# AbeelLab/phasm

Measured on AMD Instinct MI355X. Metric: overlaps_per_sec, higher is better.
Workload: dtype u64

## Files before the change

### include/phasm_overlap.h

```cpp
#ifndef PHASM_OVERLAP_H
#define PHASM_OVERLAP_H

#include <stddef.h>
#include <stdint.h>

#ifdef __cplusplus
extern "C" {
#endif

#define PO_ABI_VERSION 4

typedef enum {
    PO_OK = 0,
    PO_ERR_INVALID = 1,
    PO_ERR_NOMEM = 2,
    PO_ERR_HIP = 3,
    PO_ERR_CAPACITY = 4
} po_status;

typedef struct po_handle po_handle;
typedef struct po_result po_result;

typedef struct {
    uint32_t a_idx, b_idx;
// ... 417 lines not shown
    uint64_t n_invalid;
    uint64_t n_excluded;
    uint64_t n_root_starts;
    uint64_t n_late_starts;
    uint64_t n_blocked;
    uint64_t n_covered_edges, n_uncovered_edges;
    uint64_t n_paths;
    uint64_t n_short_paths;
    uint64_t n_isolated;
    uint64_t n_short_isolated;
    uint64_t n_contigs;
    uint64_t max_path_nodes;
    uint64_t n_chains;
    uint32_t n_path_rounds, n_cover_rounds;
    uint32_t n_batches;
    uint32_t reserved;
    float ms_ranks, ms_bubblechains, ms_paths, ms_cover, ms_label, ms_total;
} po_contig_stats;

po_status po_layout_contigs(po_handle* h, po_result* graph, const po_contig_params* params, const uint8_t* exclude_in,
                            uint32_t* edge_contig_out, uint32_t* edge_pos_out, po_contig* contigs_out, uint64_t* n_contigs_out);
po_status po_get_contig_stats(const po_handle* h, po_contig_stats* out);


typedef struct {
    uint32_t ploidy;
    uint32_t n_paths;
    uint32_t n_cands;
    uint32_t n_reads;
    uint32_t n_b;
    uint32_t start_of_block;
    uint32_t min_spanning_reads;
    uint32_t prune;
    uint32_t max_candidates;
    uint32_t n_levels;
    double threshold;
    uint32_t reserved;
    uint32_t reserved2;
} po_phase_params;

typedef struct {
    const int32_t* overlap_max;
    const uint32_t* aln_off;
    const uint32_t* aln_b;
    const int32_t* aln_a0;
    const int32_t* aln_a1;
    const uint32_t* path_off;
    const uint32_t* path_ids;
    const uint32_t* set_off;
    const uint32_t* set_ids;
    const double* levels;
} po_phase_input;

typedef struct {
    uint64_t n_extensions;
    uint64_t n_kept;
    uint64_t n_survivors;
    uint64_t level_counts[16];
    double max_rl;
    int32_t level_used;
    uint32_t n_levels;
    float ms_intervals, ms_table, ms_extend, ms_filter, ms_prune, ms_total;
} po_phase_stats;

po_status po_phase_branch(po_handle* h, const po_phase_params* params, const po_phase_input* input, uint32_t* cand_out,
                          uint32_t* ext_out, double* rl_out, uint64_t cap, double* table_out, uint64_t* n_out);
po_status po_get_phase_stats(const po_handle* h, po_phase_stats* out);


typedef struct {
    uint32_t b;
    int32_t a0, a1;
    uint32_t seq;
} po_alignment;

typedef struct {
    uint64_t n_rows, n_keys, max_degree, n_invalid;
    float ms_insert, ms_fill, ms_place, ms_total;
} po_phase_index_stats;

po_status po_phase_index(po_handle* h, po_result* rows, po_result** index_out);
po_status po_phase_index_copy(po_result* index, uint64_t* off_out, po_alignment* entries_out, uint64_t cap, uint64_t* n_out);
po_status po_get_phase_index_stats(const po_handle* h, po_phase_index_stats* out);

typedef struct {
    uint32_t mode;
    uint32_t min_spanning_reads;
    uint32_t reserved, reserved2;
} po_relevant_params;

typedef struct {
    const uint32_t* cur_graph;     uint64_t n_cur_graph;
    const uint32_t* prev_graph;    uint64_t n_prev_graph;
    const uint32_t* prev_aligning; uint64_t n_prev_aligning;
    const uint32_t* pred_read; const int32_t* pred_edge_len; uint64_t n_pred;
} po_relevant_input;

typedef struct {
    uint64_t n_cur_aligning, n_spanning, n_relevant, n_alignments, n_b;
    uint32_t fell_back, reserved;
} po_relevant_dims;

typedef struct {
    uint64_t n_cur_aligning, n_spanning, n_relevant, n_alignments, n_b;
    uint32_t fell_back, reserved;
    float ms_mark, ms_lists, ms_alignments, ms_total;
} po_relevant_stats;

po_status po_phase_relevant(po_handle* h, po_result* index, const po_relevant_params* params, const po_relevant_input* input,
                            po_result** out);
po_status po_relevant_sizes(const po_result* out, po_relevant_dims* sizes);
po_status po_relevant_copy(po_result* out, uint32_t* cur_aligning, uint32_t* rel_reads, int32_t* overlap_max, uint32_t* aln_off,
                           uint32_t* aln_b, int32_t* aln_a0, int32_t* aln_a1, uint32_t* b_reads);
po_status po_get_relevant_stats(const po_handle* h, po_relevant_stats* out);

typedef struct {
    uint64_t n_seqs, n_pieces;
    const uint64_t* seq_off;
    const uint32_t* piece_read;
    const uint32_t* piece_take;
} po_spell_input;

typedef struct {
    uint64_t n_seqs, n_pieces, n_bytes;
    uint64_t n_patched;
    float device_ms;
    uint32_t reserved;
} po_spell_stats;

po_status po_spell(po_handle* h, const po_spell_input* in, po_result** out);
po_status po_spell_sizes(const po_result* out, uint64_t* n_seqs, uint64_t* n_bytes);
po_status po_spell_copy(po_result* out, uint64_t* seq_byte_off, uint8_t* bytes, uint64_t cap);
po_status po_get_spell_stats(const po_handle* h, po_spell_stats* out);

po_status po_graph_from_edges(po_handle* h, const po_edge* edges, uint64_t n_edges, const uint32_t* node_order,
                              uint64_t n_order, po_result** out);

po_status po_result_node_order(po_result* r, uint32_t* nodes_out, uint64_t cap, uint64_t* n_out);

typedef struct {
    uint64_t n_rows;
    float ms_first_contained;
    float ms_rank;
    float ms_total;
} po_node_order_stats;
po_status po_get_node_order_stats(const po_handle* h, po_node_order_stats* out);

uint64_t po_debug_host_ranges(uint64_t* out, uint64_t cap_entries);
uint64_t po_debug_store_words(const po_handle* h, int store, const uint64_t** words);
int po_debug_expand_records(const po_cand* records, uint64_t n, const uint32_t* lengths, uint32_t n_reads, uint32_t paired,
                            po_row* rows_out, uint64_t n_rows_expected);
int po_debug_expand_packed(const uint64_t* records, uint64_t n, uint32_t sh_b, uint32_t sh_p, const uint32_t* lengths, uint32_t n_reads,
                           uint32_t paired, po_row* rows_out, uint64_t n_rows_expected);
int po_debug_fault_backtrace(int fd);
int po_debug_pointer_info(const void* p, int32_t* hip_type, int32_t* hsa_type, uint64_t* base, uint64_t* bytes);

po_status po_get_stats(const po_handle* h, po_stats* out);
const char* po_last_error(const po_handle* h);
int po_abi_version(void);

#ifdef __cplusplus
}
#endif
#endif
```

### phasm_amd/_lib.py

```python
from __future__ import annotations

import ctypes
import os

import numpy as np

HERE = os.path.dirname(os.path.abspath(__file__))
LIB_PATH = os.environ.get("PHASM_LIB") or os.path.join(HERE, "libphasm_overlap.so")

PO_OK, PO_ERR_INVALID, PO_ERR_NOMEM, PO_ERR_HIP, PO_ERR_CAPACITY = range(5)

ROW_DTYPE = np.dtype([("a_idx", "<u4"), ("b_idx", "<u4"), ("astart", "<i4"),
                      ("aend", "<i4"), ("bstart", "<i4"), ("bend", "<i4")])


CAND_DTYPE = np.dtype([("a_idx", "<u4"), ("p", "<u4"), ("b_idx", "<u4"), ("type", "<u4")])


EDGE_DTYPE = np.dtype([("u", "<u4"), ("v", "<u4"), ("weight", "<i4"), ("overlap_len", "<i4")])
COVERAGE_DTYPE = np.dtype([("read_length_sum", "<u8"), ("path_length", "<i8")])
COMPONENT_DTYPE = np.dtype([("first_node", "<u4"), ("n_nodes", "<u4"), ("n_edges", "<u8")])
SCC_DTYPE = np.dtype([("first_node", "<u4"), ("n_nodes", "<u4"), ("n_edges", "<u8"), ("n_r_in", "<u4"), ("n_re_out", "<u4")])
PART_R_IN, PART_RE_OUT, PART_START, PART_SINK = 1, 2, 4, 8
SUPERBUBBLE_DTYPE = np.dtype([("entrance", "<u4"), ("exit", "<u4"), ("n_inside", "<u4"), ("nested", "<u4")])
# ... 237 lines not shown
        return {name: getattr(self, name) for name, _ in self._fields_ if name != "reserved"}


class PoSpellInput(ctypes.Structure):
    _fields_ = [("n_seqs", ctypes.c_uint64), ("n_pieces", ctypes.c_uint64), ("seq_off", ctypes.c_void_p), ("piece_read", ctypes.c_void_p),
                ("piece_take", ctypes.c_void_p)]


class PoSpellStats(ctypes.Structure):
    _fields_ = [(name, ctypes.c_uint64) for name in ("n_seqs", "n_pieces", "n_bytes", "n_patched")] + \
               [("device_ms", ctypes.c_float), ("reserved", ctypes.c_uint32)]

    def as_dict(self) -> dict:
        return {name: getattr(self, name) for name, _ in self._fields_ if name != "reserved"}


class PoNodeOrderStats(ctypes.Structure):
    _fields_ = [("n_rows", ctypes.c_uint64), ("ms_first_contained", ctypes.c_float), ("ms_rank", ctypes.c_float),
                ("ms_total", ctypes.c_float)]

    def as_dict(self) -> dict:
        return {name: getattr(self, name) for name, _ in self._fields_}


class PoStats(ctypes.Structure):
    _fields_ = [
        ("bits_per_base", ctypes.c_uint32), ("kmer", ctypes.c_uint32),
        ("paired", ctypes.c_uint32), ("wide_index", ctypes.c_uint32),
        ("n_reads", ctypes.c_uint64), ("n_eligible", ctypes.c_uint64),
        ("total_bases", ctypes.c_uint64), ("shard_bases", ctypes.c_uint64),
        ("n_tiles", ctypes.c_uint64), ("n_candidates", ctypes.c_uint64),
        ("n_verified", ctypes.c_uint64), ("n_rows", ctypes.c_uint64),
        ("sum_overlap_bases", ctypes.c_uint64), ("verify_bytes_algo", ctypes.c_uint64),
        ("ms_index", ctypes.c_float), ("ms_scan_count", ctypes.c_float),
        ("ms_scan_fill", ctypes.c_float), ("ms_verify", ctypes.c_float),
        ("ms_select", ctypes.c_float), ("ms_emit", ctypes.c_float),
        ("ms_total", ctypes.c_float), ("ms_upload", ctypes.c_float),
        ("ms_scan_probe", ctypes.c_float), ("ms_verify_kernel", ctypes.c_float),
        ("verify_bytes_exec", ctypes.c_uint64), ("dp_steps", ctypes.c_uint64), ("dp_stopped", ctypes.c_uint64),
        ("max_diff", ctypes.c_uint32), ("band", ctypes.c_uint32), ("index_reused", ctypes.c_uint32),
        ("dp_lanes", ctypes.c_uint32), ("upload_bytes", ctypes.c_uint64),
        ("streamed", ctypes.c_uint32), ("n_deferred", ctypes.c_uint32),
        ("fused_tail", ctypes.c_uint32), ("tail_fallback", ctypes.c_uint32),
        ("n_predicted", ctypes.c_uint32), ("home_record_bytes", ctypes.c_uint32),
    ]

    def as_dict(self) -> dict:
        return {name: getattr(self, name) for name, _ in self._fields_}


_P = ctypes.c_void_p
SYMBOLS = [
    ("po_abi_version", ctypes.c_int, []),
    ("po_create", ctypes.c_int, [ctypes.POINTER(_P)]),
    ("po_destroy", None, [_P]),
    ("po_set_device", ctypes.c_int, [_P, ctypes.c_int]),
    ("po_add_sequence", ctypes.c_int, [_P, ctypes.c_char_p, ctypes.c_size_t, ctypes.c_char_p, ctypes.c_size_t]),
    ("po_add_fasta", ctypes.c_int, [_P, ctypes.c_char_p, ctypes.c_int, ctypes.POINTER(ctypes.c_uint64)]),
    ("po_num_sequences", ctypes.c_uint32, [_P]),
    ("po_get_id", ctypes.c_int, [_P, ctypes.c_uint32, ctypes.POINTER(ctypes.c_void_p), ctypes.POINTER(ctypes.c_size_t)]),
    ("po_get_length", ctypes.c_uint32, [_P, ctypes.c_uint32]),
    ("po_upload", ctypes.c_int, [_P]),
    ("po_invalidate", ctypes.c_int, [_P]),
    ("po_upload_piece", ctypes.c_int, [_P, ctypes.c_uint32, ctypes.c_uint32, ctypes.c_void_p, ctypes.c_uint64,
                                       ctypes.POINTER(ctypes.c_uint64), ctypes.POINTER(ctypes.c_int)]),
    ("po_upload_assemble", ctypes.c_int, [_P, ctypes.c_void_p, ctypes.c_uint64, ctypes.c_uint32]),
    ("po_upload_piece_part", ctypes.c_int, [_P, ctypes.c_uint32, ctypes.c_uint32, ctypes.c_uint32, ctypes.c_uint32, ctypes.c_void_p,
                                            ctypes.c_uint64, ctypes.POINTER(ctypes.c_uint64), ctypes.POINTER(ctypes.c_int)]),
    ("po_upload_assemble_parts", ctypes.c_int, [_P, ctypes.c_void_p, ctypes.c_uint64, ctypes.c_uint32, ctypes.c_uint32]),
    ("po_overlaps", ctypes.c_int, [_P, ctypes.c_uint32, ctypes.POINTER(_P)]),
    ("po_overlaps_to_host", ctypes.c_int, [_P, ctypes.c_uint32, ctypes.POINTER(_P)]),
    ("po_overlaps_ex", ctypes.c_int, [_P, ctypes.c_uint32, ctypes.c_uint32, ctypes.c_uint32, ctypes.POINTER(_P)]),
    ("po_overlaps_shard", ctypes.c_int, [_P, ctypes.c_uint32, ctypes.c_uint32, ctypes.c_uint32, ctypes.POINTER(_P)]),
    ("po_candidates_shard", ctypes.c_int, [_P, ctypes.c_uint32, ctypes.c_uint32, ctypes.c_uint32, ctypes.POINTER(_P)]),
    ("po_expand", ctypes.c_int, [_P, ctypes.c_void_p, ctypes.c_uint64, ctypes.POINTER(_P)]),
    ("po_candidates_shard_into", ctypes.c_int, [_P, ctypes.c_uint32, ctypes.c_uint32, ctypes.c_uint32, ctypes.c_void_p,
                                               ctypes.c_uint64, ctypes.POINTER(ctypes.c_int), ctypes.POINTER(_P)]),
    ("po_index_slice_build", ctypes.c_int, [_P, ctypes.c_uint32, ctypes.c_uint32, ctypes.c_uint32, ctypes.POINTER(ctypes.c_uint32),
                                            ctypes.POINTER(ctypes.c_uint32), ctypes.POINTER(ctypes.c_uint64)]),
    ("po_index_chunk_bytes", ctypes.c_uint64, [ctypes.c_uint32, ctypes.c_uint64, ctypes.POINTER(ctypes.c_uint64)]),
    ("po_index_slice_export", ctypes.c_int, [_P, ctypes.c_void_p, ctypes.c_uint64]),
    ("po_candidates_shard_indexed", ctypes.c_int, [_P, ctypes.c_uint32, ctypes.c_uint32, ctypes.c_uint32, ctypes.c_void_p, ctypes.c_uint32,
                                                   ctypes.c_uint32, ctypes.c_uint64, ctypes.c_void_p, ctypes.c_uint64,
                                                   ctypes.POINTER(ctypes.c_int), ctypes.POINTER(_P)]),
    ("po_overlaps_shard_indexed", ctypes.c_int, [_P, ctypes.c_uint32, ctypes.c_uint32, ctypes.c_uint32, ctypes.c_void_p, ctypes.c_uint32,
                                                 ctypes.c_uint32, ctypes.c_uint64, ctypes.POINTER(_P)]),
    ("po_shard_range", ctypes.c_int, [_P, ctypes.c_uint32, ctypes.c_uint32, ctypes.POINTER(ctypes.c_uint32), ctypes.POINTER(ctypes.c_uint32)]),
    ("po_result_count", ctypes.c_uint64, [_P]),
    ("po_result_rows", ctypes.c_void_p, [_P]),
    ("po_result_rows_range", ctypes.c_void_p, [_P, ctypes.c_uint64, ctypes.c_uint64]),
    ("po_result_device_rows", ctypes.c_void_p, [_P]),
    ("po_result_copy_to_device", ctypes.c_int, [_P, ctypes.c_void_p]),
    ("po_result_copy_prefix_to_device", ctypes.c_int, [_P, ctypes.c_void_p, ctypes.c_uint64]),
    ("po_result_free", None, [_P]),
    ("po_write_gfa_edges", ctypes.c_int, [_P, ctypes.c_int, ctypes.POINTER(ctypes.c_uint64)]),
    ("po_write_gfa_segments", ctypes.c_int, [_P, ctypes.c_int, ctypes.POINTER(ctypes.c_uint64)]),
    ("po_add_segment", ctypes.c_int, [_P, ctypes.c_char_p, ctypes.c_size_t, ctypes.c_uint32]),
    ("po_result_from_rows", ctypes.c_int, [_P, ctypes.c_void_p, ctypes.c_uint64, ctypes.POINTER(_P)]),
    ("po_add_gfa", ctypes.c_int, [_P, ctypes.c_char_p, ctypes.POINTER(ctypes.c_uint64), ctypes.POINTER(_P)]),
    ("po_layout_edges", ctypes.c_int, [_P, _P, ctypes.POINTER(PoLayoutParams), ctypes.c_void_p, ctypes.POINTER(_P)]),
    ("po_get_layout_stats", ctypes.c_int, [_P, ctypes.POINTER(PoLayoutStats)]),
    ("po_layout_reduce", ctypes.c_int, [_P, _P, ctypes.POINTER(PoReduceParams), ctypes.c_void_p, ctypes.POINTER(_P)]),
    ("po_get_reduce_stats", ctypes.c_int, [_P, ctypes.POINTER(PoReduceStats)]),
    ("po_layout_tips", ctypes.c_int, [_P, _P, ctypes.POINTER(PoTipsParams), ctypes.c_void_p, ctypes.POINTER(_P)]),
    ("po_get_tips_stats", ctypes.c_int, [_P, ctypes.POINTER(PoTipsStats)]),
    ("po_layout_diamonds", ctypes.c_int, [_P, _P, ctypes.POINTER(PoDiamondParams), ctypes.c_void_p, ctypes.POINTER(_P)]),
    ("po_get_diamond_stats", ctypes.c_int, [_P, ctypes.POINTER(PoDiamondStats)]),
    ("po_layout_merge", ctypes.c_int, [_P, _P, ctypes.POINTER(PoMergeParams), ctypes.c_void_p, ctypes.POINTER(_P)]),
    ("po_get_merge_stats", ctypes.c_int, [_P, ctypes.POINTER(PoMergeStats)]),
    ("po_result_merged_paths", ctypes.c_int, [_P, ctypes.POINTER(ctypes.c_uint64), ctypes.POINTER(ctypes.c_uint64), ctypes.c_void_p,
                                              ctypes.c_uint64, ctypes.c_void_p, ctypes.c_void_p, ctypes.c_uint64, ctypes.c_void_p]),
    ("po_layout_coverage", ctypes.c_int, [_P, _P, _P, ctypes.POINTER(PoCoverageParams), ctypes.c_void_p]),
    ("po_get_coverage_stats", ctypes.c_int, [_P, ctypes.POINTER(PoCoverageStats)]),
    ("po_layout_components", ctypes.c_int, [_P, _P, ctypes.POINTER(PoComponentsParams), ctypes.c_void_p, ctypes.c_void_p, ctypes.c_void_p,
                                            ctypes.POINTER(ctypes.c_uint64)]),
    ("po_get_components_stats", ctypes.c_int, [_P, ctypes.POINTER(PoComponentsStats)]),
    ("po_layout_partition", ctypes.c_int, [_P, _P, ctypes.POINTER(PoPartitionParams), ctypes.c_void_p, ctypes.c_void_p, ctypes.c_void_p,
                                           ctypes.c_void_p, ctypes.POINTER(ctypes.c_uint64)]),
    ("po_get_partition_stats", ctypes.c_int, [_P, ctypes.POINTER(PoPartitionStats)]),
    ("po_layout_superbubbles", ctypes.c_int, [_P, _P, ctypes.POINTER(PoSuperbubbleParams), ctypes.c_void_p, ctypes.c_void_p, ctypes.c_void_p,
                                              ctypes.c_void_p, ctypes.POINTER(ctypes.c_uint64)]),
    ("po_get_superbubble_stats", ctypes.c_int, [_P, ctypes.POINTER(PoSuperbubbleStats)]),
    ("po_layout_bubblechains", ctypes.c_int, [_P, _P, ctypes.POINTER(PoBubblechainParams), ctypes.c_void_p, ctypes.c_void_p, ctypes.c_void_p,
                                              ctypes.c_void_p, ctypes.POINTER(ctypes.c_uint64)]),
    ("po_get_bubblechain_stats", ctypes.c_int, [_P, ctypes.POINTER(PoBubblechainStats)]),
    ("po_layout_contigs", ctypes.c_int, [_P, _P, ctypes.POINTER(PoContigParams), ctypes.c_void_p, ctypes.c_void_p, ctypes.c_void_p,
                                         ctypes.c_void_p, ctypes.POINTER(ctypes.c_uint64)]),
    ("po_get_contig_stats", ctypes.c_int, [_P, ctypes.POINTER(PoContigStats)]),
    ("po_phase_branch", ctypes.c_int, [_P, ctypes.POINTER(PoPhaseParams), ctypes.POINTER(PoPhaseInput), ctypes.c_void_p, ctypes.c_void_p,
                                       ctypes.c_void_p, ctypes.c_uint64, ctypes.c_void_p, ctypes.POINTER(ctypes.c_uint64)]),
    ("po_get_phase_stats", ctypes.c_int, [_P, ctypes.POINTER(PoPhaseStats)]),
    ("po_phase_index", ctypes.c_int, [_P, _P, ctypes.POINTER(_P)]),
    ("po_phase_index_copy", ctypes.c_int, [_P, ctypes.c_void_p, ctypes.c_void_p, ctypes.c_uint64, ctypes.POINTER(ctypes.c_uint64)]),
    ("po_get_phase_index_stats", ctypes.c_int, [_P, ctypes.POINTER(PoPhaseIndexStats)]),
    ("po_phase_relevant", ctypes.c_int, [_P, _P, ctypes.POINTER(PoRelevantParams), ctypes.POINTER(PoRelevantInput), ctypes.POINTER(_P)]),
    ("po_relevant_sizes", ctypes.c_int, [_P, ctypes.POINTER(PoRelevantDims)]),
    ("po_relevant_copy", ctypes.c_int, [_P] + [ctypes.c_void_p] * 8),
    ("po_get_relevant_stats", ctypes.c_int, [_P, ctypes.POINTER(PoRelevantStats)]),
    ("po_spell", ctypes.c_int, [_P, ctypes.POINTER(PoSpellInput), ctypes.POINTER(_P)]),
    ("po_spell_sizes", ctypes.c_int, [_P, ctypes.POINTER(ctypes.c_uint64), ctypes.POINTER(ctypes.c_uint64)]),
    ("po_spell_copy", ctypes.c_int, [_P, ctypes.c_void_p, ctypes.c_void_p, ctypes.c_uint64]),
    ("po_get_spell_stats", ctypes.c_int, [_P, ctypes.POINTER(PoSpellStats)]),
    ("po_graph_from_edges", ctypes.c_int, [_P, ctypes.c_void_p, ctypes.c_uint64, ctypes.c_void_p, ctypes.c_uint64, ctypes.POINTER(_P)]),
    ("po_result_node_order", ctypes.c_int, [_P, ctypes.c_void_p, ctypes.c_uint64, ctypes.POINTER(ctypes.c_uint64)]),
    ("po_get_node_order_stats", ctypes.c_int, [_P, ctypes.POINTER(PoNodeOrderStats)]),
    ("po_get_stats", ctypes.c_int, [_P, ctypes.POINTER(PoStats)]),
    ("po_last_error", ctypes.c_char_p, [_P]),
    ("po_debug_fault_backtrace", ctypes.c_int, [ctypes.c_int]),
    ("po_debug_store_words", ctypes.c_uint64, [_P, ctypes.c_int, ctypes.POINTER(ctypes.c_void_p)]),
    ("po_debug_expand_packed", ctypes.c_int, [ctypes.c_void_p, ctypes.c_uint64, ctypes.c_uint32, ctypes.c_uint32, ctypes.c_void_p, ctypes.c_uint32,
                                              ctypes.c_uint32, ctypes.c_void_p, ctypes.c_uint64]),
    ("po_debug_expand_records", ctypes.c_int, [ctypes.c_void_p, ctypes.c_uint64, ctypes.c_void_p, ctypes.c_uint32, ctypes.c_uint32,
                                               ctypes.c_void_p, ctypes.c_uint64]),
    ("po_debug_host_ranges", ctypes.c_uint64, [ctypes.POINTER(ctypes.c_uint64), ctypes.c_uint64]),
    ("po_debug_pointer_info", ctypes.c_int, [ctypes.c_void_p, ctypes.POINTER(ctypes.c_int32), ctypes.POINTER(ctypes.c_int32),
                                             ctypes.POINTER(ctypes.c_uint64), ctypes.POINTER(ctypes.c_uint64)]),
]

_lib = None


def _preload_torch_hip_runtime() -> None:
    import importlib.util
    if os.environ.get("PHASM_HIP_RUNTIME") == "system":
        return
    try:
        spec = importlib.util.find_spec("torch")
    except (ImportError, ValueError):
        spec = None
    if spec is None or not spec.submodule_search_locations:
        return
    path = os.path.join(list(spec.submodule_search_locations)[0], "lib", "libamdhip64.so")
    if os.path.exists(path):
        try:
            ctypes.CDLL(path, mode=ctypes.RTLD_GLOBAL)
        except OSError:
            pass


def load() -> ctypes.CDLL:
    global _lib
    if _lib is None:
        _preload_torch_hip_runtime()
        if not os.path.exists(LIB_PATH):
            raise ImportError(
                "%s not found: build it with `python -m phasm_amd.build` (hipcc, gfx950). "
                "phasm_amd has no CPU fallback." % LIB_PATH)
        lib = ctypes.CDLL(LIB_PATH)
        for name, restype, argtypes in SYMBOLS:
            fn = getattr(lib, name)
            fn.restype = restype
            fn.argtypes = argtypes
        _lib = lib
    return _lib
```

### phasm_amd/csrc/c_api.hip

```cpp
#include "../../include/phasm_overlap.h"

#include <hip/hip_runtime.h>

#include <dlfcn.h>
#include <execinfo.h>
#include <fcntl.h>
#include <signal.h>
#include <sys/mman.h>
#include <sys/stat.h>
#include <unistd.h>

#include <algorithm>
#include <array>
#include <atomic>
#include <chrono>
#include <cmath>
#include <condition_variable>
#include <cstdio>
#include <cstdlib>
#include <cstring>
#include <deque>
#include <functional>
#include <memory>
#include <mutex>
#include <new>
#include <string>
#include <system_error>
#include <thread>
#include <unordered_map>
#include <vector>

#include "kernels.hip.h"
#include "extend.hip.h"
#include "layout.hip.h"
#include "reduce.hip.h"
#include "tips.hip.h"
#include "diamond.hip.h"
#include "merge.hip.h"
#include "coverage.hip.h"
#include "components.hip.h"
#include "partition.hip.h"
#include "superbubbles.hip.h"
#include "bubblechains.hip.h"
#include "contigs.hip.h"
#include "phase.hip.h"
#include "relevant.hip.h"
#include "spell.hip.h"

namespace {

enum { RB_CNT, RB_DEG, RB_OFF, RB_CUR, RB_TKEY, RB_TTGT, RB_TEID, RB_CTGT, RB_CW, RB_CEID, RB_CIDPOS, RB_STGT, RB_SEID, RB_STATE,
       RB_FLAG1, RB_FLAGS, RB_KEEP, RB_KOFF, RB_N };
enum { TB_CNT, TB_OUTDEG, TB_OUTSUM, TB_INDEG, TB_INSUM, TB_MARK, TB_CAND, TB_CSTATE, TB_EFLAG, TB_FLAGS, TB_KEEP, TB_KOFF,
       TB_TKEY, TB_TVAL, TB_ALIVE, TB_RCNT, TB_N };
enum { MB_CNT, MB_RCNT, MB_OUTDEG, MB_INDEG, MB_OUTE, MB_INE, MB_LINK, MB_BACK, MB_JB0, MB_JB1, MB_HOPS0, MB_HOPS1, MB_WS0, MB_WS1,
       MB_HKEY, MB_HVAL, MB_HLEN, MB_HSUM, MB_PATHK, MB_LENS, MB_PSUM, MB_NPATH, MB_NPOS, MB_EFLAG, MB_KEEP, MB_KOFF, MB_TMP, MB_LEN,
       MB_N };
enum { VB_CNT, VB_USED, VB_NODEOF, VB_LEN, VB_TABLE, VB_SUM, VB_SETCNT, VB_OFF, VB_CUR, VB_LIST, VB_OUT, VB_N };
enum { RK_CNT, RK_RCNT, RK_KEY, RK_VAL, RK_RANKOF, RK_ENDS, RK_ROOT, RK_INDEX, RK_N };
enum { KB_P, KB_COMP, KB_ECOMP, KB_TABLE, KB_N };
enum { PB_LIVE, PB_SCC, PB_COLOUR, PB_MARK, PB_HASIN, PB_HASOUT, PB_NODESCC, PB_FLAGW, PB_FLAGS, PB_ECLASS, PB_TABLE, PB_N };
enum { UB_CNT, UB_W, UB_CIN, UB_COUT, UB_OFFIN, UB_OFFOUT, UB_CURIN, UB_CUROUT, UB_LISTIN, UB_LISTOUT, UB_LVLF, UB_LVLB, UB_IDOM, UB_IPDOM,
       UB_DEPTH, UB_EXIT, UB_ENCL, UB_INSIDE, UB_TOTAL, UB_DEAD, UB_EXITOUT, UB_INSIDEOUT, UB_FLAGSOUT, UB_TABLE, UB_N };
enum { HB_CNT, HB_FW, HB_NEXT, HB_PRED, HB_TOP, HB_JB0, HB_JB1, HB_HOPS0, HB_HOPS1, HB_NHEAD, HB_NPOS, HB_CB, HB_CN, HB_LAST, HB_CE,
       HB_CHAINOUT, HB_BUBBLEOUT, HB_EDGEOUT, HB_TABLE, HB_N };
enum { CB_CNT, CB_EXCL, CB_LEN, CB_INDEG, CB_OUTDEG, CB_INE, CB_NLEN, CB_CLS, CB_JB0, CB_JB1, CB_HOPS0, CB_HOPS1, CB_WS0, CB_WS1, CB_CJ0,
       CB_CJ1, CB_OK0, CB_OK1, CB_HEADOF, CB_PN, CB_PLAST, CB_PLEN, CB_KEPT, CB_KEY, CB_VAL, CB_CONTIGOUT, CB_POSOUT, CB_TABLE, CB_N };
enum { FB_CNT, FB_HIST, FB_LEVELS, FB_OM, FB_ALNOFF, FB_ALNB, FB_A0, FB_A1, FB_POFF, FB_PIDS, FB_SOFF, FB_SIDS, FB_SBITS, FB_PBITS, FB_SIV,
       FB_PIV, FB_TABLE, FB_RL, FB_KEEP, FB_PLACE, FB_KCAND, FB_KEXT, FB_KRL, FB_KEEP2, FB_PLACE2, FB_SCAND, FB_SEXT, FB_SRL, FB_N };
enum { XB_CNT, XB_DEG, XB_CUR, XB_TMP, XB_EX, XB_LISTS, XB_BITS, XB_WCNT, XB_WRANK, XB_CA, XB_REL, XB_B, XB_ALNCNT, XB_ALNOFF, XB_OM,
       XB_ALNB, XB_A0, XB_A1, XB_N };
enum { SB_IN, SB_SCAN, SB_POFF, SB_SOFF, SB_N };
constexpr int EV_LAY_N = 83;
enum { EV_EDGES = 0, EV_REDUCE = 4, EV_TIPS = 9, EV_NODE_ORDER = 15, EV_DIAMONDS = 18, EV_MERGE = 22, EV_COVERAGE = 27, EV_COMPONENTS = 30,
       EV_PARTITION = 34, EV_SUPERBUBBLES = 38, EV_BUBBLECHAINS = 45, EV_CONTIGS = 54, EV_PHASE = 67, EV_PHASE_INDEX = 73,
       EV_RELEVANT = 77, EV_SPELL = 81 };
static_assert(EV_BUBBLECHAINS + 9 == EV_CONTIGS, "po_layout_bubblechains has nine events");
static_assert(EV_CONTIGS + 13 == EV_PHASE, "po_layout_contigs has thirteen events");
static_assert(EV_PHASE + 6 == EV_PHASE_INDEX, "po_phase_branch has six events");
static_assert(EV_PHASE_INDEX + 4 == EV_RELEVANT, "po_phase_index has four events");
static_assert(EV_RELEVANT + 4 == EV_SPELL, "po_phase_relevant has four events");
static_assert(EV_SPELL + 2 == EV_LAY_N, "the two events of po_spell are the last of the layout events");
constexpr int TIP_BATCH = 24;

struct DevBuf {
    void* p = nullptr;
    size_t cap = 0;
    bool arena = false;
    template <typename T> T* as() const { return static_cast<T*>(p); }
    void release() {
        if (p && !arena) (void)hipFree(p);
        p = nullptr;
        cap = 0;
        arena = false;
    }
};

struct PinNote {
    uint64_t base, bytes;
    uint32_t kind;
};
std::mutex g_pin_mu;
std::vector<PinNote> g_pins;
uint64_t g_pins_ever = 0;
constexpr size_t PIN_LOG_MAX = 1u << 16;
void pin_note(const void* p, size_t bytes, uint32_t kind) {
    if (!p) return;
    std::lock_guard<std::mutex> lock(g_pin_mu);
    ++g_pins_ever;
    for (PinNote& n : g_pins)
        if (n.base == (uint64_t)(uintptr_t)p && n.bytes == bytes && (n.kind & 0xFFu) == kind) {
            n.kind |= 0x100u;
            return;
        }
    if (g_pins.size() < PIN_LOG_MAX) g_pins.push_back(PinNote{(uint64_t)(uintptr_t)p, (uint64_t)bytes, kind | 0x100u});
}
void pin_drop(const void* p) {
    if (!p) return;
    std::lock_guard<std::mutex> lock(g_pin_mu);
    for (PinNote& n : g_pins)
        if (n.base == (uint64_t)(uintptr_t)p && (n.kind & 0x100u)) n.kind &= ~0x100u;
}

struct HostBuf {
    void* p = nullptr;
    size_t cap = 0;
    void release() {
        if (p) {
            pin_drop(p);
            (void)hipHostFree(p);
        }
        p = nullptr;
        cap = 0;
    }
};

inline int phase_events_env() {
    if (const char* e = getenv("PHASM_PHASE_EVENTS")) {
        const int v = atoi(e);
        return v == 1 ? 1 : v == 2 ? 2 : 0;
    }
    return getenv("PHASM_STREAM_TRACE") ? 1 : -1;
}
enum { EV_START = 0, EV_INDEX, EV_COUNT, EV_FILL, EV_VERIFY, EV_SELECT, EV_EMIT, EV_PROBE0, EV_PROBE1, EV_VER0, EV_VER1, EV_DONE, EV_N };

}

constexpr int PO_MAX_PIECES = 16;

struct RegHeader {
    size_t bytes;
    int registered;
};
constexpr size_t REG_PAGE = 4096;
thread_local bool g_reg_defer = false;
template <class T>
struct RegAlloc {
    using value_type = T;
    RegAlloc() = default;
    template <class U> RegAlloc(const RegAlloc<U>&) {}
    T* allocate(size_t n) {
        const size_t bytes = ((n * sizeof(T) + REG_PAGE - 1) / REG_PAGE) * REG_PAGE;
        void* base = nullptr;
        if (posix_memalign(&base, REG_PAGE, bytes + REG_PAGE) != 0 || !base) throw std::bad_alloc();
        RegHeader* hd = static_cast<RegHeader*>(base);
        hd->bytes = bytes;
        hd->registered = 0;
        char* data = static_cast<char*>(base) + REG_PAGE;
        if (getenv("PHASM_POISON_HOST")) std::memset(data, 0xA5, bytes);
        if (!g_reg_defer) reg_now(data);
        return reinterpret_cast<T*>(data);
    }
    static void reg_now(void* data) {
        RegHeader* hd = reinterpret_cast<RegHeader*>(static_cast<char*>(data) - REG_PAGE);
        if (hd->registered || hd->bytes < (1u << 20) || getenv("PHASM_NO_PIN")) return;
        if (hipHostRegister(data, hd->bytes, hipHostRegisterPortable) == hipSuccess) {
            hd->registered = 1;
            pin_note(data, hd->bytes, 2u);
        } else {
            (void)hipGetLastError();
        }
    }
    template <class U> void construct(U*) noexcept {}
    template <class U, class A0, class... Args> void construct(U* q, A0&& a0, Args&&... args) {
        ::new (static_cast<void*>(q)) U(std::forward<A0>(a0), std::forward<Args>(args)...);
    }
    void deallocate(T* p, size_t) {
        char* base = reinterpret_cast<char*>(p) - REG_PAGE;
        RegHeader* hd = reinterpret_cast<RegHeader*>(base);
        if (hd->registered) {
            pin_drop(p);
            (void)hipHostUnregister(p);
        }
        free(base);
    }
    template <class U> bool operator==(const RegAlloc<U>&) const { return true; }
    template <class U> bool operator!=(const RegAlloc<U>&) const { return false; }
};
using WordStore = std::vector<uint64_t, RegAlloc<uint64_t>>;
inline bool store_is_pinned(const WordStore& w) {
    if (w.capacity() == 0) return false;
    const RegHeader* hd = reinterpret_cast<const RegHeader*>(reinterpret_cast<const char*>(w.data()) - REG_PAGE);
    return hd->registered != 0;
}
constexpr size_t STAGE_MAX = 4u << 20;

struct po_handle {
    int device = 0;
    bool dev_ready = false;
    hipStream_t stream = nullptr;
    hipEvent_t ev_sets[2][EV_N] = {};
    hipEvent_t* ev = ev_sets[0];
    hipEvent_t ev_up0 = nullptr, ev_up1 = nullptr;
    uint64_t* pinned = nullptr;
    uint64_t* pinned_dev = nullptr;
    int n_cu = 256;
    size_t lds_max = 64 * 1024;
    std::string err;

    int bits = 2;
    std::vector<std::string> ids;
    std::vector<uint32_t> len;
    std::vector<uint64_t> cum_len;
    std::vector<uint64_t> woff;
    WordStore words[2];
    bool all_pairs_rc = true;
    bool all_pairs_rcx = true;
    uint64_t base1 = 0;
    uint64_t dev_words = 0;
    uint64_t upload_bytes = 0;
    std::vector<uint32_t> exc_off{0};
    std::vector<uint32_t> exc_pos;
    std::vector<uint8_t> exc_byte;
    std::vector<uint8_t> pair_state;
    uint64_t total_bases = 0;
    bool dirty = true;

    DevBuf d_words, d_woff, d_len, d_tiles, d_read_tile0, d_exc_off, d_exc_pos, d_exc_byte, d_pair_state;
    std::vector<uint32_t> h_read_tile0;
    uint32_t n_tiles = 0;
    uint32_t max_len = 0;
    size_t n_exc_uploaded = 0;
    bool paired = false;

    DevBuf d_table, d_slot_cnt, d_slot_cur, d_slot_start, d_read_slot, d_chain, d_chain_tmp, d_long_list;
    DevBuf d_entry_off;
    DevBuf d_bloom, d_selfrep, d_tile_count, d_tile_off, d_truemask, d_ps_blocks, d_scalars, d_left, d_left_cnt, d_tile_extra;
    DevBuf d_cand_a, d_cand_p, d_cand_b, d_type, d_rowcnt, d_row_off, d_flag, d_pair_key, d_pair_min;
    DevBuf d_vlabel, d_vrank, d_vperm;
    DevBuf d_chain_state;
    DevBuf d_tail_state;
    DevBuf spare_rows;
    DevBuf spare_cands;
    DevBuf spare_edges;
    DevBuf spare_nrank;
    DevBuf spare_spell;
    HostBuf spare_host;
    HostBuf scratch_host;
    uint64_t pool_bases = 0;
    std::vector<void*> arena_chunks;
    char* arena_cur = nullptr;
    size_t arena_left = 0;
    int poison = -1;
    hipStream_t copy_stream = nullptr;
    DevBuf chunk_rows[PO_MAX_PIECES + 1];
    bool chunk_compact[PO_MAX_PIECES + 1] = {};
    bool home_on = false;
    HostBuf home_stage;
    size_t home_used = 0;
    uint64_t home_seq = 0;
    uint32_t home_gen = 0;
    uint32_t home_sh_b = 0, home_sh_p = 0;
    uint64_t home_pack_n = ~0ull, home_pack_bases = ~0ull;
    uint32_t home_pack_b = 0, home_pack_p = 0;
    uint64_t home_last_bytes = 0;

    hipStream_t up_stream = nullptr;
    hipEvent_t ev_piece[PO_MAX_PIECES] = {};
    hipStream_t rc_stream = nullptr;
    hipEvent_t ev_rc[PO_MAX_PIECES] = {};
    hipEvent_t ev_meta = nullptr;
    hipEvent_t ev_first = nullptr;
    WordStore first_words;
    uint32_t first_n = 0;
    WordStore lead_words;
    uint32_t lead_n = 0;
    uint32_t st_lead = 2;
    HostBuf meta_host;
    HostBuf stage_host;
    size_t stage_used = 0;
    uint32_t meta_n = 0xFFFFFFFFu;
    int meta_bits = 0;
    uint64_t elig_n = ~0ull, elig_val = 0;
    uint32_t elig_m = 0;
    DevBuf d_first, d_defer;
    uint32_t defer_need = 0;
    struct Pending {
        bool valid = false;
        uint32_t k = 0;
        po_stats S = {};
        bool ver_timed = false;
// ... 207 lines not shown
    if (!h->dev_ready) return;
    (void)hipSetDevice(h->device);
    (void)hipStreamSynchronize(h->stream);
    if (h->up_stream) (void)hipStreamSynchronize(h->up_stream);
    if (h->rc_stream) (void)hipStreamSynchronize(h->rc_stream);
}

po_status init_device(po_handle* h);

inline bool home_enabled() {
    const char* e = getenv("PHASM_HOME");
    return !(e && atoi(e) == 0);
}

void result_pool_grow(po_handle* h, uint64_t bases = 0) {
    if (!bases) bases = h->total_bases;
    h->pool_bases = bases + bases / 2;
    if (getenv("PHASM_NO_POOL")) return;
    if (!h->dev_ready && init_device(h) != PO_OK) h->err.clear();
    const uint64_t want = std::min<uint64_t>(h->pool_bases / 160 * sizeof(po_row), 4ull << 30);
    if (h->spare_host.cap >= want || h->live_results) return;
    int n = 0;
    if (hipGetDeviceCount(&n) != hipSuccess || n == 0) {
        (void)hipGetLastError();
        h->pool_bases = ~0ull;
        return;
    }
    AllocTrace tr("result pool", want);
    h->spare_host.release();
    if (hipHostMalloc(&h->spare_host.p, want, hipHostMallocPortable) == hipSuccess) {
        h->spare_host.cap = want;
        pin_note(h->spare_host.p, want, 1u);
        if (home_enabled() && h->home_stage.cap < want / 3) (void)ensure_host(h, h->home_stage, want / 3);
        if (h->dev_ready && h->up_stream && h->copy_stream && want >= (16u << 20) && !getenv("PHASM_NO_WARM")) {
            void* w = nullptr;
            const size_t nb = 8u << 20;
            if (hipMalloc(&w, nb) == hipSuccess) {
                (void)hipMemcpyAsync(w, h->spare_host.p, nb, hipMemcpyHostToDevice, h->up_stream);
                (void)hipStreamSynchronize(h->up_stream);
                (void)hipMemcpyAsync(static_cast<char*>(h->spare_host.p) + nb, w, nb, hipMemcpyDeviceToHost, h->copy_stream);
                (void)hipStreamSynchronize(h->copy_stream);
                (void)hipFree(w);
            }
            (void)hipGetLastError();
        }
    } else {
        (void)hipGetLastError();
        h->spare_host.p = nullptr;
        h->pool_bases = ~0ull;
    }
}

#define PO_TRY(expr)                    \
    do {                                \
        po_status s_ = (expr);          \
        if (s_ != PO_OK) return s_;     \
    } while (0)

struct DevKit {
    int device = -1;
    hipStream_t stream = nullptr, copy_stream = nullptr, up_stream = nullptr, rc_stream = nullptr;
    hipEvent_t ev_sets[2][EV_N] = {};
    hipEvent_t ev_up0 = nullptr, ev_up1 = nullptr, ev_meta = nullptr, ev_first = nullptr;
    hipEvent_t ev_piece[PO_MAX_PIECES] = {}, ev_rc[PO_MAX_PIECES] = {}, ev_lay[EV_LAY_N] = {};

    uint64_t* pinned = nullptr;
    uint64_t* pinned_dev = nullptr;
};
static_assert(sizeof(DevKit::ev_lay) == sizeof(po_handle::ev_lay), "a kit carries every layout event of a handle");
std::mutex g_kit_mu;
std::vector<DevKit> g_kits;
constexpr size_t KIT_POOL_MAX = 8;

bool kit_take(po_handle* h) {
    std::lock_guard<std::mutex> lock(g_kit_mu);
    for (size_t i = 0; i < g_kits.size(); ++i) {
        if (g_kits[i].device != h->device) continue;
        const DevKit k = g_kits[i];
        g_kits.erase(g_kits.begin() + (long)i);
        h->stream = k.stream;
        h->copy_stream = k.copy_stream;
        h->up_stream = k.up_stream;
        h->rc_stream = k.rc_stream;
        std::memcpy(h->ev_sets, k.ev_sets, sizeof(k.ev_sets));
        h->ev_up0 = k.ev_up0;
        h->ev_up1 = k.ev_up1;
        h->ev_meta = k.ev_meta;
        h->ev_first = k.ev_first;
        std::memcpy(h->ev_piece, k.ev_piece, sizeof(k.ev_piece));
        std::memcpy(h->ev_rc, k.ev_rc, sizeof(k.ev_rc));
        std::memcpy(h->ev_lay, k.ev_lay, sizeof(k.ev_lay));
        h->pinned = k.pinned;
        h->pinned_dev = k.pinned_dev;
        return true;
    }
    return false;
}

bool kit_give(po_handle* h) {
    if (getenv("PHASM_NO_KIT_POOL") || !h->stream || !h->copy_stream || !h->up_stream || !h->rc_stream || !h->pinned) return false;
    if (hipStreamSynchronize(h->stream) != hipSuccess || hipStreamSynchronize(h->copy_stream) != hipSuccess ||
        hipStreamSynchronize(h->up_stream) != hipSuccess || hipStreamSynchronize(h->rc_stream) != hipSuccess) {
        (void)hipGetLastError();
        return false;
    }
    DevKit k;
    k.device = h->device;
    k.stream = h->stream;
    k.copy_stream = h->copy_stream;
    k.up_stream = h->up_stream;
    k.rc_stream = h->rc_stream;
    std::memcpy(k.ev_sets, h->ev_sets, sizeof(k.ev_sets));
    k.ev_up0 = h->ev_up0;
    k.ev_up1 = h->ev_up1;
    k.ev_meta = h->ev_meta;
    k.ev_first = h->ev_first;
    std::memcpy(k.ev_piece, h->ev_piece, sizeof(k.ev_piece));
    std::memcpy(k.ev_rc, h->ev_rc, sizeof(k.ev_rc));
    std::memcpy(k.ev_lay, h->ev_lay, sizeof(k.ev_lay));
    k.pinned = h->pinned;
    k.pinned_dev = h->pinned_dev;
    std::lock_guard<std::mutex> lock(g_kit_mu);
    if (g_kits.size() >= KIT_POOL_MAX) return false;
    g_kits.push_back(k);
    return true;
}


unsigned cpu_share() {
    static const unsigned share = [] {
        unsigned n = std::thread::hardware_concurrency();
        n = n ? n : 4u;
        long long q = -1, per = 100000;
        if (FILE* f = std::fopen("/sys/fs/cgroup/cpu.max", "r")) {
            char buf[64] = {0};
            if (std::fscanf(f, "%63s %lld", buf, &per) >= 1 && std::strcmp(buf, "max") != 0) q = atoll(buf);
            std::fclose(f);
        } else if (FILE* g = std::fopen("/sys/fs/cgroup/cpu/cpu.cfs_quota_us", "r")) {
            if (std::fscanf(g, "%lld", &q) != 1) q = -1;
            std::fclose(g);
            if (FILE* g2 = std::fopen("/sys/fs/cgroup/cpu/cpu.cfs_period_us", "r")) {
                if (std::fscanf(g2, "%lld", &per) != 1) per = 100000;
                std::fclose(g2);
            }
        }
        if (q > 0 && per > 0) n = std::min<unsigned>(n, (unsigned)std::max<long long>(1, q / per));
        return n;
    }();
    return share;
}

namespace home {

constexpr uint32_t CHUNK = 4096;

struct Job {
    const void* rec = nullptr;
    uint32_t sh_b = 0, sh_p = 0;
    uint64_t n_rec = 0;
    po_row* out = nullptr;
    uint64_t n_rows = 0;
    const volatile uint32_t* flag = nullptr;
    uint32_t want = 0;
    uint32_t paired = 0, bits = 2;
};

struct Pool {
    std::vector<std::thread> thr;
    std::mutex mu;
    std::condition_variable cv_queue;
    std::condition_variable cv_job;
    std::mutex call_mu;
    std::deque<Job> queue;
    std::atomic<uint64_t> submitted{0}, finished{0};
    std::atomic<int> error{0};
    const uint32_t* len = nullptr;
    uint32_t n_reads = 0;
    std::atomic<uint64_t> sum_l{0}, sum_b{0}, sum_e{0};
    Job cur;
    uint64_t job_seq = 0;
    uint32_t n_chunks = 0;
    std::vector<uint64_t> chunk_off;
    std::atomic<uint32_t> next_count{0}, done_count{0}, next_write{0}, done_write{0};
    std::atomic<int> phase{0};
    std::atomic<int> inside{0};
    std::chrono::steady_clock::time_point t0;
    std::vector<std::array<double, 3>> trace;
    bool tracing = false;
};

Pool* g_pool = nullptr;
std::once_flag g_pool_once;

inline void cpu_pause() {
#if defined(__x86_64__) || defined(__i386__)
    __builtin_ia32_pause();
#endif
}

std::atomic<uint32_t> g_spin_limit{4096};
template <class Pred>
inline void spin_until(Pred pred) {
    const uint32_t limit = g_spin_limit.load(std::memory_order_relaxed);
    for (uint32_t n = 0; !pred(); ++n) {
        if (limit == 0 || n < limit) cpu_pause();
        else std::this_thread::yield();
    }
}

inline po::Cand load_rec(const Job& j, uint64_t i) {
    if (!j.sh_b) return static_cast<const po::Cand*>(j.rec)[i];
    return po::unpack_record(static_cast<const uint64_t*>(j.rec)[i], j.sh_b, j.sh_p);
}

inline uint32_t rows_of_rec(const po::Cand& c, uint32_t paired) {
    if (!paired) return (c.type & 1u) + ((c.type >> 1) & 1u);
    return ((c.type & 1u) ? (c.a == (c.b ^ 1u) ? 1u : 2u) : 0u) + ((c.type & 2u) ? 2u : 0u);
}

inline void put_row(uint64_t*& o, uint32_t a, uint32_t b, uint32_t astart, uint32_t aend, uint32_t bend) {
    __builtin_nontemporal_store((uint64_t)a | ((uint64_t)b << 32), o);
    __builtin_nontemporal_store((uint64_t)astart | ((uint64_t)aend << 32), o + 1);
    __builtin_nontemporal_store((uint64_t)bend << 32, o + 2);
    o += 3;
}

bool expand_records(Pool& P, uint64_t lo, uint64_t hi, po_row* out) {
    uint64_t* o = reinterpret_cast<uint64_t*>(out);
    const Job& job = P.cur;
    const uint32_t* len = P.len;
    const uint32_t paired = job.paired, n_reads = P.n_reads, bits = job.bits;
    auto pb = [bits](uint32_t l) -> uint64_t { return bits == 8u ? l : (l >> 2) + ((l & 3u) != 0u); };
    uint64_t sl = 0, sb = 0, se = 0;
    for (uint64_t i = lo; i < hi; ++i) {
        const po::Cand c = load_rec(job, i);
        if (c.a >= n_reads || c.b >= n_reads) return false;
        const uint32_t la = len[c.a], lb = len[c.b];
        se += 2 * pb((c.type & 1u) ? la - c.p : lb);
        if (c.type & 1u) {
            const uint32_t l = la - c.p;
            const bool twin = paired && c.a != (c.b ^ 1u);
            put_row(o, c.a, c.b, c.p, la, l);
            if (twin) put_row(o, c.b ^ 1u, c.a ^ 1u, lb - l, lb, l);
            const uint64_t k = twin ? 2 : 1;
            sl += k * l;
            sb += k * 2 * pb(l);
        }
        if (c.type & 2u) {
            put_row(o, c.a, c.b, c.p, c.p + lb, lb);
            if (paired) put_row(o, c.a ^ 1u, c.b ^ 1u, la - c.p - lb, la - c.p, lb);
            const uint64_t k = paired ? 2 : 1;
            sl += k * lb;
            sb += k * 2 * pb(lb);
        }
    }
    P.sum_l.fetch_add(sl, std::memory_order_relaxed);
    P.sum_b.fetch_add(sb, std::memory_order_relaxed);
    P.sum_e.fetch_add(se, std::memory_order_relaxed);
    return true;
}

void run_phases(Pool& P, bool lead) {
    const uint32_t nc = P.n_chunks;
    for (;;) {
        const uint32_t c = P.next_count.fetch_add(1, std::memory_order_relaxed);
        if (c >= nc) break;
        const uint64_t lo = (uint64_t)c * CHUNK, hi = std::min<uint64_t>(P.cur.n_rec, lo + CHUNK);
        uint64_t n = 0;
        const uint32_t paired = P.cur.paired;
        for (uint64_t i = lo; i < hi; ++i) n += rows_of_rec(load_rec(P.cur, i), paired);
        P.chunk_off[c + 1] = n;
        P.done_count.fetch_add(1, std::memory_order_release);
    }
    if (lead) {
        spin_until([&] { return P.done_count.load(std::memory_order_acquire) >= nc; });
        P.chunk_off[0] = 0;
        for (uint32_t c = 0; c < nc; ++c) P.chunk_off[c + 1] += P.chunk_off[c];
        if (P.chunk_off[nc] != P.cur.n_rows) P.error.store(1);
        P.phase.store(P.error.load() ? 0 : 2, std::memory_order_release);
    } else {
        spin_until([&] { return P.phase.load(std::memory_order_acquire) != 1; });
    }
    if (P.phase.load(std::memory_order_acquire) != 2) return;
    for (;;) {
        const uint32_t c = P.next_write.fetch_add(1, std::memory_order_relaxed);
        if (c >= nc) break;
        const uint64_t lo = (uint64_t)c * CHUNK, hi = std::min<uint64_t>(P.cur.n_rec, lo + CHUNK);
        if (!expand_records(P, lo, hi, P.cur.out + P.chunk_off[c])) P.error.store(2);
#if defined(__x86_64__)
        __builtin_ia32_sfence();
#endif
        P.done_write.fetch_add(1, std::memory_order_release);
    }
}

void helper(Pool* Pp) {
    Pool& P = *Pp;
    uint64_t seen = 0;
    for (;;) {
        {
            std::unique_lock<std::mutex> lock(P.mu);
            P.cv_job.wait(lock, [&] { return P.job_seq != seen; });
            seen = P.job_seq;
        }
        P.inside.fetch_add(1, std::memory_order_acq_rel);
        if (P.phase.load(std::memory_order_acquire) != 0) run_phases(P, false);
        P.inside.fetch_sub(1, std::memory_order_release);
    }
}

void leader(Pool* Pp) {
    Pool& P = *Pp;
    for (;;) {
        Job j;
        {
            std::unique_lock<std::mutex> lock(P.mu);
            P.cv_queue.wait(lock, [&] { return !P.queue.empty(); });
            j = P.queue.front();
            P.queue.pop_front();
        }
        if (j.flag)
            spin_until([&] { return *j.flag == j.want; });
        std::atomic_thread_fence(std::memory_order_acquire);
        const double t_ready = P.tracing ? std::chrono::duration<double, std::micro>(std::chrono::steady_clock::now() - P.t0).count() : 0.0;
        if (P.error.load() == 0 && j.n_rec) {
            spin_until([&] { return P.inside.load(std::memory_order_acquire) == 0; });
            P.cur = j;
            P.n_chunks = (uint32_t)((j.n_rec + CHUNK - 1) / CHUNK);
            if (P.chunk_off.size() < (size_t)P.n_chunks + 1) P.chunk_off.resize((size_t)P.n_chunks + 1);
            P.next_count.store(0);
            P.done_count.store(0);
            P.next_write.store(0);
            P.done_write.store(0);
            P.phase.store(1, std::memory_order_release);
            {
                std::lock_guard<std::mutex> lock(P.mu);
                ++P.job_seq;
            }
            P.cv_job.notify_all();
            run_phases(P, true);
            if (P.phase.load() == 2)
                spin_until([&] { return P.done_write.load(std::memory_order_acquire) >= P.n_chunks; });
            P.phase.store(0, std::memory_order_release);
            std::atomic_thread_fence(std::memory_order_seq_cst);
        }
        if (P.tracing)
            P.trace.push_back({t_ready, std::chrono::duration<double, std::micro>(std::chrono::steady_clock::now() - P.t0).count(), (double)j.n_rows});
        P.finished.fetch_add(1, std::memory_order_release);
    }
}

Pool* pool() {
    std::call_once(g_pool_once, [] {
        Pool* P = new Pool();
        unsigned n = cpu_share();
        n = std::max(1u, std::min(n * 3 / 4, 12u));
        if (const char* e = getenv("PHASM_HOME_THREADS")) n = (unsigned)std::max(1, std::min(64, atoi(e)));
        try {
            P->thr.emplace_back(leader, P);
            P->thr.back().detach();
            for (unsigned i = 1; i < n; ++i) {
                P->thr.emplace_back(helper, P);
                P->thr.back().detach();
            }
        } catch (const std::system_error&) {
        }
        if (P->thr.empty()) {
            delete P;
            P = nullptr;
        }
        g_pool = P;
    });
    return g_pool;
}

void begin(Pool* P, const uint32_t* len, uint32_t n_reads, bool tracing) {
    if (const char* e = getenv("PHASM_HOME_SPIN")) g_spin_limit.store((uint32_t)std::max(0, atoi(e)));
    else g_spin_limit.store(4096);
    P->len = len;
    P->n_reads = n_reads;
    P->error.store(0);
    P->submitted.store(0);
    P->finished.store(0);
    P->sum_l.store(0);
    P->sum_b.store(0);
    P->sum_e.store(0);
    P->tracing = tracing;
    P->trace.clear();
    P->t0 = std::chrono::steady_clock::now();
}

void submit(Pool* P, const Job& j) {
    {
        std::lock_guard<std::mutex> lock(P->mu);
        P->queue.push_back(j);
    }
    P->submitted.fetch_add(1, std::memory_order_release);
    P->cv_queue.notify_one();
}

void wait_all(Pool* P) {
    spin_until([&] { return P->finished.load(std::memory_order_acquire) >= P->submitted.load(std::memory_order_acquire); });
}

}

po_status init_device(po_handle* h) {
    if (h->dev_ready) {
        HIP_TRY(h, hipSetDevice(h->device));
        return PO_OK;
    }
    AllocTrace tr("init_device", 0);
    const auto ti0 = std::chrono::steady_clock::now();
    auto imark = [&](const char* what) {
        if (tr.on) std::fprintf(stderr, "[init] %s at %.1f ms\n", what, std::chrono::duration<double, std::milli>(std::chrono::steady_clock::now() - ti0).count());
    };
    int n = 0;
    hipError_t e = hipGetDeviceCount(&n);
    imark("runtime up (hipGetDeviceCount)");
    if (e != hipSuccess || n == 0)
        return fail(h, PO_ERR_HIP, "no HIP device available (libphasm_overlap has no CPU fallback)");
    if (h->device < 0 || h->device >= n) return fail(h, PO_ERR_INVALID, "device ordinal out of range");
    HIP_TRY(h, hipSetDevice(h->device));
    hipDeviceProp_t prop;
    HIP_TRY(h, hipGetDeviceProperties(&prop, h->device));
    h->n_cu = prop.multiProcessorCount > 0 ? prop.multiProcessorCount : 256;
    h->lds_max = prop.sharedMemPerBlock;
    if (const char* e = getenv("PHASM_POISON")) h->poison = (int)(strtol(e, nullptr, 0) & 0xFF);
    if (!getenv("PHASM_NO_KIT_POOL") && kit_take(h)) {
        h->ev = h->ev_sets[0];
        std::memset(h->pinned, 0, 1024);
        hipLaunchKernelGGL(po::k_fill_u32, dim3(1), dim3(64), 0, h->stream, reinterpret_cast<uint32_t*>(h->pinned_dev + 63), (uint64_t)1, 0u);
        (void)hipGetLastError();
        h->dev_ready = true;
        return PO_OK;
    }
    imark("device selected, properties read");
    HIP_TRY(h, hipStreamCreateWithFlags(&h->stream, hipStreamNonBlocking));
    imark("first stream made");
    for (int i = 0; i < 2 * EV_N; ++i) HIP_TRY(h, hipEventCreate(&h->ev_sets[i / EV_N][i % EV_N]));
    HIP_TRY(h, hipEventCreate(&h->ev_up0));
    HIP_TRY(h, hipEventCreate(&h->ev_up1));
    imark("first events made");
    HIP_TRY(h, hipHostMalloc(reinterpret_cast<void**>(&h->pinned), 1024, hipHostMallocDefault));
    pin_note(h->pinned, 1024, 1u);
    HIP_TRY(h, hipHostGetDevicePointer(reinterpret_cast<void**>(&h->pinned_dev), h->pinned, 0));
    imark("landing zone made");
    if (const char* e = getenv("PHASM_POISON")) h->poison = (int)(strtol(e, nullptr, 0) & 0xFF);
    HIP_TRY(h, hipStreamCreateWithFlags(&h->copy_stream, hipStreamNonBlocking));
    imark("copy stream made");
    HIP_TRY(h, hipStreamCreateWithFlags(&h->up_stream, hipStreamNonBlocking));
    HIP_TRY(h, hipStreamCreateWithFlags(&h->rc_stream, hipStreamNonBlocking));
    imark("other streams made");
    for (int k = 0; k < PO_MAX_PIECES; ++k) {
        HIP_TRY(h, hipEventCreate(&h->ev_piece[k]));
        HIP_TRY(h, hipEventCreateWithFlags(&h->ev_rc[k], hipEventDisableTiming));
    }
    HIP_TRY(h, hipEventCreateWithFlags(&h->ev_first, hipEventDisableTiming));
    HIP_TRY(h, hipEventCreateWithFlags(&h->ev_meta, hipEventDisableTiming));
    imark("streams and events made");
    hipLaunchKernelGGL(po::k_fill_u32, dim3(1), dim3(64), 0, h->stream, reinterpret_cast<uint32_t*>(h->pinned_dev + 63), (uint64_t)1, 0u);
    (void)hipGetLastError();
    imark("first launch queued (code object loaded)");
    if (!getenv("PHASM_NO_WARM")) {
        void* w = nullptr;
        if (hipMalloc(&w, 256) == hipSuccess) {
            uint32_t* wd = static_cast<uint32_t*>(w);
            (void)hipMemcpyAsync(wd, h->pinned + 62, 8, hipMemcpyHostToDevice, h->up_stream);
            hipLaunchKernelGGL(po::k_fill_u32, dim3(1), dim3(64), 0, h->up_stream, wd + 8, (uint64_t)1, 0u);
            (void)hipMemcpyAsync(wd + 16, h->pinned + 62, 8, hipMemcpyHostToDevice, h->stream);
            hipLaunchKernelGGL(po::k_fill_u32, dim3(1), dim3(64), 0, h->rc_stream, wd + 24, (uint64_t)1, 0u);
            hipLaunchKernelGGL(po::k_fill_u32, dim3(1), dim3(64), 0, h->copy_stream, wd + 32, (uint64_t)1, 0u);
            (void)hipMemcpyAsync(h->pinned + 61, wd + 32, 8, hipMemcpyDeviceToHost, h->copy_stream);
            (void)hipMemcpyAsync(h->pinned + 60, wd + 16, 8, hipMemcpyDeviceToHost, h->stream);
            (void)hipStreamSynchronize(h->up_stream);
            (void)hipStreamSynchronize(h->rc_stream);
            (void)hipStreamSynchronize(h->copy_stream);
            (void)hipStreamSynchronize(h->stream);
            (void)hipFree(w);
        }
        (void)hipGetLastError();
        imark("queues and copy paths warmed");
        static const void* const warm_kernels[] = {
            (const void*)po::k_abs_woff, (const void*)po::k_build_tiles, (const void*)po::k_revcomp_store, (const void*)po::k_scatter_first,
            (const void*)po::k_paired_check, (const void*)po::k_call_init, (const void*)po::k_call_reset, (const void*)po::k_table_insert,
            (const void*)po::k_chain_fill, (const void*)po::k_chain_sort_short<uint32_t>, (const void*)po::k_chain_sort_long<uint32_t>,
            (const void*)po::k_table_finalize, (const void*)po::k_ps_reduce<uint32_t>, (const void*)po::k_ps_spine, (const void*)po::k_ps_down<uint32_t>,
            (const void*)po::k_ps_reduce<uint8_t>, (const void*)po::k_ps_down<uint8_t>, (const void*)po::k_ps_chain<uint32_t>,
            (const void*)po::k_ps_chain<uint8_t>, (const void*)po::k_ps_small,
            (const void*)po::k_scan_probe<2, true, true>, (const void*)po::k_scan_probe<2, true, false>, (const void*)po::k_scan_fixup<2, true>,
            (const void*)po::k_scan_fixup<2, false>, (const void*)po::k_scan_fill<2, true>, (const void*)po::k_scan_fill<2, false>,
            (const void*)po::k_read_label, (const void*)po::k_read_sort, (const void*)po::k_read_invert, (const void*)po::k_defer_split,
            (const void*)po::k_verify_a<2, false, true, true>, (const void*)po::k_verify_a<2, false, true, false>,
            (const void*)po::k_verify_a<2, true, true, false>, (const void*)po::k_select_local, (const void*)po::k_tile_rows<true>,
            (const void*)po::k_tile_rows<false>, (const void*)po::k_tail, (const void*)po::k_tail_cands, (const void*)po::k_select,
            (const void*)po::k_emit, (const void*)po::k_verify_flat, (const void*)po::k_deferred_rowcnt, (const void*)po::k_emit_cands,
            (const void*)po::k_wide_insert<2, 1>, (const void*)po::k_wide_insert<2, 16>, (const void*)po::k_wide_chain_fill<2, 1>,
            (const void*)po::k_wide_chain_fill<2, 16>, (const void*)po::k_wide_finalize<2, 1>, (const void*)po::k_wide_finalize<2, 16>,
            (const void*)po::k_chain_sort_short<uint64_t>, (const void*)po::k_chain_sort_long<uint64_t>,
            (const void*)po::k_wide_scan<2, false, true, 1>, (const void*)po::k_wide_scan<2, true, true, 1>,
            (const void*)po::k_wide_scan<2, false, false, 16>, (const void*)po::k_wide_scan<2, true, false, 16>};
        for (const void* k : warm_kernels) {
            hipFuncAttributes fa;
            (void)hipFuncGetAttributes(&fa, k);
        }
        (void)hipGetLastError();
        imark("kernels looked up");
    }
    h->dev_ready = true;
    return PO_OK;
}

struct BaseLut {
    uint8_t v[256];
    BaseLut() {
        std::memset(v, 0x80, sizeof(v));
        v[(unsigned char)'A'] = 0;
        v[(unsigned char)'C'] = 1;
        v[(unsigned char)'G'] = 2;
        v[(unsigned char)'T'] = 3;
    }
};
const BaseLut g_lut;

bool append_packed(po_handle* h, const unsigned char* s, size_t n, int bits) {
    const size_t per = 64 / bits;
    WordStore& store = h->words[h->woff.size() & 1];
    const size_t old_size = store.size();
    const size_t off = (old_size + 1) & ~size_t(1);
    const size_t nw = (n + per - 1) / per;
    store.resize(off + nw + 1, 0);
    uint64_t* w = store.data() + off;
    if (bits == 2) {
        const uint8_t* lut = g_lut.v;
        uint8_t bad = 0;
        const size_t full = n / 32;
        for (size_t k = 0; k < full; ++k) {
            const unsigned char* q = s + k * 32;
            uint64_t acc = 0;
            for (int j = 0; j < 32; ++j) {
                const uint8_t c = lut[q[j]];
                bad |= c;
                acc |= (uint64_t)(c & 3) << (2 * j);
            }
            w[k] = acc;
        }
        if (full * 32 < n) {
            uint64_t acc = 0;
            for (size_t i = full * 32; i < n; ++i) {
                const uint8_t c = lut[s[i]];
                bad |= c;
                acc |= (uint64_t)(c & 3) << (2 * (i & 31));
            }
            w[full] = acc;
        }
        if (bad & 0x80) {
            size_t cnt = 0;
            for (size_t i = 0; i < n; ++i) cnt += lut[s[i]] >> 7;
            if (cnt > n / 64 + 16) {
                store.resize(old_size);
                return false;
            }
            for (size_t i = 0; i < n; ++i) {
                if (lut[s[i]] & 0x80) {
                    h->exc_pos.push_back((uint32_t)i);
                    h->exc_byte.push_back(s[i]);
                }
            }
        }
        h->exc_off.push_back((uint32_t)h->exc_pos.size());
    } else {
        for (size_t i = 0; i < n; ++i) w[i >> 3] |= (uint64_t)s[i] << ((i & 7) * 8);
    }
    h->woff.push_back(off);
    return true;
}

void materialize(const po_handle* h, size_t r, const WordStore* stores, const uint64_t* woff, std::vector<unsigned char>& out) {
    const uint32_t n = h->len[r];
    out.resize(n);
    const uint64_t* w = stores[r & 1].data() + woff[r];
    for (uint32_t i = 0; i < n; ++i) out[i] = "ACGT"[(w[i >> 5] >> ((i & 31) * 2)) & 3];
    for (uint32_t e = h->exc_off[r]; e < h->exc_off[r + 1]; ++e) out[h->exc_pos[e]] = h->exc_byte[e];
}

void widen_to_bytes(po_handle* h) {
    WordStore old_words[2];
    std::vector<uint64_t> old_off;
    old_words[0].swap(h->words[0]);
    old_words[1].swap(h->words[1]);
    old_off.swap(h->woff);
    std::vector<unsigned char> tmp;
    for (size_t r = 0; r < h->len.size(); ++r) {
        materialize(h, r, old_words, old_off.data(), tmp);
        append_packed(h, tmp.data(), h->len[r], 8);
    }
    h->bits = 8;
    h->all_pairs_rc = false;
    h->all_pairs_rcx = false;
    h->first_n = 0;
    h->first_words.clear();
    h->lead_n = 0;
    h->lead_words.clear();
    h->exc_off.assign(1, 0);
    h->exc_pos.clear();
    h->exc_byte.clear();
    h->pair_state.clear();
}

const unsigned char* comp_table() {
    static unsigned char comp[256];
    static bool init = false;
    if (!init) {
        for (int i = 0; i < 256; ++i) comp[i] = (unsigned char)i;
        const char* from = "ACGTURYKMBVDHSWNacgturykmbvdhswn";
        const char* to = "TGCAAYRMKVBHDSWNtgcaayrmkvbhdswn";
        for (int i = 0; from[i]; ++i) comp[(unsigned char)from[i]] = (unsigned char)to[i];
        init = true;
    }
    return comp;
}

void host_pair_check(po_handle* h, size_t r, const unsigned char* s) {
    const size_t pair = r / 2;
    if (h->pair_state.size() <= pair) h->pair_state.resize(pair + 1, 0);
    const bool has_exc = h->exc_off[r - 1] != h->exc_off[r] || h->exc_off[r] != h->exc_off[r + 1];
    if (!has_exc) return;
    const uint32_t n = h->len[r];
    uint8_t state = 1;
    if (h->len[r - 1] != n) {
        state = 2;
    } else {
        std::vector<unsigned char> prev;
        materialize(h, r - 1, h->words, h->woff.data(), prev);
        const unsigned char* c = comp_table();
        for (uint32_t i = 0; i < n; ++i) {
            const unsigned char x = prev[n - 1 - i], y = s[i];
            if (c[x] != y || c[y] != x) {
                state = 2;
                break;
            }
        }
    }
    h->pair_state[pair] = state;
}

bool packed_is_revcomp(const po_handle* h, size_t r) {
    const uint32_t L = h->len[r];
    if (h->len[r - 1] != L) return false;
// ... 4160 lines not shown
    } catch (const std::bad_alloc&) {
        st = fail(h, PO_ERR_NOMEM, "out of host memory in po_upload_assemble");
    }
    h->asm_pieces = nullptr;
    h->asm_parts = 1;
    if (st != PO_OK && h->dev_ready) (void)hipStreamSynchronize(h->stream);
    if (st == PO_OK) {
        h->upload_bytes += piece_bytes;
        h->stats.upload_bytes = h->upload_bytes;
    }
    return st;
}

po_status po_upload_assemble(po_handle* h, const void* pieces_device, uint64_t slot_words, uint32_t nshards) {
    return po_upload_assemble_parts(h, pieces_device, slot_words, nshards, 1);
}

po_status po_invalidate(po_handle* h) {
    if (!h) return PO_ERR_INVALID;
    h->dirty = true;
    return PO_OK;
}

static po_status overlaps_common(po_handle* h, const OverlapArgs& a, po_result** out, void* ext_dst = nullptr, uint64_t ext_cap = 0) {
    if (!h || !out) return PO_ERR_INVALID;
    *out = nullptr;
    if (a.nshards == 0 || a.shard >= a.nshards) return fail(h, PO_ERR_INVALID, "shard must be < nshards");
    if (h->segments_only) return fail(h, PO_ERR_INVALID, "this handle holds GFA segments without sequences: nothing to overlap");
    po_result* r = new (std::nothrow) po_result();
    if (!r) return fail(h, PO_ERR_NOMEM, "out of host memory");
    r->h = h;
    r->ext_dst = ext_dst;
    r->ext_cap = ext_cap;
    po_status st;
    try {
        st = upload(h);
        if (st == PO_OK) st = h->bits == 2 ? run_overlaps<2>(h, a, r) : run_overlaps<8>(h, a, r);
    } catch (const std::bad_alloc&) {
        st = fail(h, PO_ERR_NOMEM, "out of host memory in po_overlaps");
    }
    if (st != PO_OK) {
        if (h->dev_ready) (void)hipStreamSynchronize(h->stream);
        r->d_rows.release();
        delete r;
        return st;
    }
    ++h->live_results;
    *out = r;
    return PO_OK;
}

po_status po_overlaps_shard(po_handle* h, uint32_t min_length, uint32_t shard, uint32_t nshards, po_result** out) {
    return overlaps_common(h, OverlapArgs{min_length, shard, nshards, false}, out);
}

po_status po_candidates_shard(po_handle* h, uint32_t min_length, uint32_t shard, uint32_t nshards, po_result** out) {
    return overlaps_common(h, OverlapArgs{min_length, shard, nshards, true}, out);
}

po_status po_candidates_shard_into(po_handle* h, uint32_t min_length, uint32_t shard, uint32_t nshards, void* dst_device,
                                   uint64_t capacity, int* written, po_result** out) {
    if (written) *written = 0;
    if (!dst_device && capacity) return PO_ERR_INVALID;
    const po_status st = overlaps_common(h, OverlapArgs{min_length, shard, nshards, true}, out, dst_device, capacity);
    if (st == PO_OK && written) *written = (*out)->wrote_ext ? 1 : 0;
    return st;
}

po_status po_expand(po_handle* h, const void* candidates_device, uint64_t n_candidates, po_result** out) {
    if (!h || !out || (!candidates_device && n_candidates)) return PO_ERR_INVALID;
    *out = nullptr;
    if (h->segments_only) return fail(h, PO_ERR_INVALID, "this handle holds GFA segments without sequences");
    po_result* r = new (std::nothrow) po_result();
    if (!r) return fail(h, PO_ERR_NOMEM, "out of host memory");
    r->h = h;
    po_status st;
    try {
        st = upload(h);
        if (st == PO_OK) st = run_expand(h, candidates_device, n_candidates, r);
    } catch (const std::bad_alloc&) {
        st = fail(h, PO_ERR_NOMEM, "out of host memory in po_expand");
    }
    if (st != PO_OK) {
        if (h->dev_ready) (void)hipStreamSynchronize(h->stream);
        r->d_rows.release();
        delete r;
        return st;
    }
    ++h->live_results;
    *out = r;
    return PO_OK;
}

po_status po_overlaps(po_handle* h, uint32_t min_length, po_result** out) {
    return po_overlaps_shard(h, min_length, 0, 1, out);
}

extern "C++" {
namespace {

struct HostRows {
    HostBuf hb;
    uint64_t total = 0;
};

bool home_begin(po_handle* h) {
    h->home_on = false;
    if (!home_enabled()) return false;
    home::Pool* P = home::pool();
    if (!P) return false;
    P->call_mu.lock();
    home::begin(P, h->len.data(), (uint32_t)h->len.size(), getenv("PHASM_STREAM_TRACE") != nullptr || getenv("PHASM_HOME_TRACE") != nullptr);
    h->home_on = true;
    h->home_used = 0;
    h->home_seq = 0;
    if (h->home_pack_n != h->len.size() || h->home_pack_bases != h->total_bases) {
        uint32_t longest = 0;
        for (uint32_t l : h->len) longest = std::max(longest, l);
        uint32_t br = 1, bp = 1;
        while ((1ull << br) < (uint64_t)h->len.size()) ++br;
        while ((1ull << bp) < (uint64_t)longest + 1ull) ++bp;
        const bool fits = 2 * br + bp <= 62;
        h->home_pack_b = fits ? br : 0u;
        h->home_pack_p = fits ? 2 * br : 0u;
        h->home_pack_n = h->len.size();
        h->home_pack_bases = h->total_bases;
    }
    const char* pk = getenv("PHASM_HOME_PACK");
    const bool pack = !(pk && atoi(pk) == 0);
    h->home_sh_b = pack ? h->home_pack_b : 0u;
    h->home_sh_p = pack ? h->home_pack_p : 0u;
    return true;
}

void home_wait(po_handle* h) {
    if (h->home_on) home::wait_all(home::g_pool);
}

int home_end(po_handle* h, po_stats* sum = nullptr) {
    if (!h->home_on) return 0;
    home::Pool* P = home::g_pool;
    home::wait_all(P);
    const int err = P->error.load();
    if (sum) {
        sum->sum_overlap_bases += P->sum_l.load();
        sum->verify_bytes_algo += P->sum_b.load();
        sum->verify_bytes_exec += P->sum_e.load();
    }
    if (P->tracing)
        for (size_t i = 0; i < P->trace.size(); ++i)
            std::fprintf(stderr, "[home] piece %zu: records home at %.3f ms, %.0f rows written at %.3f ms (since the call set the pool up)\n", i,
                         P->trace[i][0] * 1e-3, P->trace[i][2], P->trace[i][1] * 1e-3);
    h->home_on = false;
    P->call_mu.unlock();
    return err;
}

po_status rows_room(po_handle* h, HostRows& R, uint64_t nk, uint32_t k, uint32_t n_chunks, double seen_share) {
    const size_t need = (size_t)(R.total + nk) * sizeof(po_row);
    if (need <= R.hb.cap) return PO_OK;
    uint64_t guess = std::max<uint64_t>(h->last_host_rows, (R.total + nk) * n_chunks / (k + 1));
    if (seen_share > 0.0) guess = std::max<uint64_t>(guess, (uint64_t)((double)(R.total + nk) / seen_share * 1.05));
    HostBuf bigger;
    PO_TRY(ensure_host(h, bigger, std::max<size_t>(need, (size_t)(guess + guess / 8) * sizeof(po_row))));
    home_wait(h);
    if (hipStreamSynchronize(h->copy_stream) != hipSuccess) {
        bigger.release();
        return fail(h, PO_ERR_HIP, "copy stream");
    }
    if (R.total) std::memcpy(bigger.p, R.hb.p, (size_t)R.total * sizeof(po_row));
    R.hb.release();
    R.hb = bigger;
    return PO_OK;
}

po_status append_home(po_handle* h, HostRows& R, const DevBuf& dev, uint64_t n_rec, uint64_t nk, uint32_t k, uint32_t n_chunks,
                      double seen_share = 0.0) {
    if (nk == 0) return PO_OK;
    home::Pool* P = home::g_pool;
    PO_TRY(rows_room(h, R, nk, k, n_chunks, seen_share));
    const size_t elem = h->home_sh_b ? sizeof(uint64_t) : sizeof(po::Cand);
    const size_t bytes = (size_t)n_rec * elem;
    constexpr uint64_t N_EV = 32;
    if (h->home_used + bytes > h->home_stage.cap || (h->home_seq && h->home_seq % N_EV == 0)) {
        home_wait(h);
        if (hipStreamSynchronize(h->copy_stream) != hipSuccess) return fail(h, PO_ERR_HIP, "copy stream");
        h->home_used = 0;
        if (bytes > h->home_stage.cap)
            PO_TRY(ensure_host(h, h->home_stage, std::max<size_t>({bytes * 2, (size_t)(h->home_last_bytes + h->home_last_bytes / 8), (size_t)8 << 20})));
    }
    const uint32_t slot = (uint32_t)(h->home_seq % N_EV);
    const uint32_t want = ++h->home_gen;
    char* dst = static_cast<char*>(h->home_stage.p) + h->home_used;
    HIP_TRY(h, hipMemcpyAsync(dst, dev.p, bytes, hipMemcpyDeviceToHost, h->copy_stream));
    hipLaunchKernelGGL(po::k_fill_u32, dim3(1), dim3(64), 0, h->copy_stream, reinterpret_cast<uint32_t*>(h->pinned_dev + 96 + slot), (uint64_t)1, want);
    HIP_TRY(h, hipGetLastError());
    home::Job j;
    j.rec = dst;
    j.sh_b = h->home_sh_b;
    j.sh_p = h->home_sh_p;
    j.n_rec = n_rec;
    j.out = static_cast<po_row*>(R.hb.p) + R.total;
    j.n_rows = nk;
    j.flag = reinterpret_cast<const volatile uint32_t*>(h->pinned + 96 + slot);
    j.want = want;
    j.paired = (h->bits == 2 && h->paired) ? 1u : 0u;
    j.bits = (uint32_t)h->bits;
    home::submit(P, j);
    ++h->home_seq;
    h->home_used += (bytes + 255) & ~size_t(255);
    h->home_last_bytes += bytes;
    R.total += nk;
    return PO_OK;
}

po_status append_rows(po_handle* h, HostRows& R, const DevBuf& dev, uint64_t nk, uint32_t k, uint32_t n_chunks, double seen_share = 0.0) {
    if (nk == 0) return PO_OK;
    PO_TRY(rows_room(h, R, nk, k, n_chunks, seen_share));
    HIP_TRY(h, hipMemcpyAsync(static_cast<char*>(R.hb.p) + (size_t)R.total * sizeof(po_row), dev.p, (size_t)nk * sizeof(po_row),
                              hipMemcpyDeviceToHost, h->copy_stream));
    R.total += nk;
    return PO_OK;
}

void add_stats(po_stats& sum, const po_stats& S) {
    sum.n_candidates += S.n_candidates;
    sum.n_verified += S.n_verified;
    sum.n_rows += S.n_rows;
    sum.sum_overlap_bases += S.sum_overlap_bases;
    sum.verify_bytes_algo += S.verify_bytes_algo;
    sum.verify_bytes_exec += S.verify_bytes_exec;
    sum.n_tiles += S.n_tiles;
    sum.shard_bases += S.shard_bases;
    sum.fused_tail += S.fused_tail;
    sum.tail_fallback += S.tail_fallback;
    sum.n_predicted += S.n_predicted;
    sum.ms_index += S.ms_index;
    sum.ms_scan_count += S.ms_scan_count;
    sum.ms_scan_fill += S.ms_scan_fill;
    sum.ms_verify += S.ms_verify;
    sum.ms_select += S.ms_select;
    sum.ms_emit += S.ms_emit;
    sum.ms_total += S.ms_total;
    sum.ms_scan_probe += S.ms_scan_probe;
    sum.ms_verify_kernel += S.ms_verify_kernel;
}

po_status run_chunk(po_handle* h, const OverlapArgs& a, uint64_t* nk) {
    const uint32_t k = a.shard;
    po_result part;
    part.h = h;
    if (h->chunk_rows[k].p) {
        h->spare_rows.release();
        h->spare_rows = h->chunk_rows[k];
        h->chunk_rows[k] = DevBuf();
    }
    const po_status st = h->bits == 2 ? run_overlaps<2>(h, a, &part) : run_overlaps<8>(h, a, &part);
    h->chunk_rows[k] = part.d_rows;
    h->chunk_compact[k] = part.compact;
    part.d_rows = DevBuf();
    *nk = part.count;
    return st;
}

bool stream_eligible(const po_handle* h, uint32_t min_length) {
    const uint32_t n = (uint32_t)h->len.size();
    if (!h->dirty || h->bits != 2 || n < 4 || (n % 2) != 0 || !h->all_pairs_rcx) return false;
    if (h->asm_pieces) return false;
    if (getenv("PHASM_FULL_UPLOAD") || getenv("PHASM_NO_MIRROR")) return false;
    bool want = n >= 4096 && h->words[0].size() * 8 >= (16ull << 20);
    if (const char* e = getenv("PHASM_STREAM")) want = atoi(e) != 0;
    if (!want) return false;
    const uint32_t m = min_length ? min_length : 1;
    const uint64_t n_elig = count_eligible(const_cast<po_handle*>(h), m);
    if (n_elig == 0) return false;
    return true;
}

std::vector<uint32_t> stream_bounds(const po_handle* h) {
    const uint32_t n = (uint32_t)h->len.size();
    const uint64_t bytes0 = (uint64_t)h->words[0].size() * 8;
    uint64_t max_pieces = h->chunk_rows[0].p ? 12 : 8;
    const bool big = bytes0 >= (512ull << 20) && h->chunk_rows[0].p;
    if (big) max_pieces = 15;
    if (const char* e = getenv("PHASM_STREAM_MAX_PIECES")) max_pieces = (uint64_t)std::max(2, std::min(PO_MAX_PIECES - 1, atoi(e)));
    const uint32_t n_pieces = (uint32_t)std::min<uint64_t>(max_pieces, std::max<uint64_t>(2, (bytes0 + (8ull << 20)) / (16ull << 20)));
    const double skew = big ? 1.6 : 1.25;
    std::vector<uint32_t> cuts;
    for (uint32_t i = 1; i < n_pieces; ++i) cuts.push_back((uint32_t)(1000.0 * (1.0 - std::pow(1.0 - (double)i / n_pieces, skew))));
    if (const char* e = getenv("PHASM_STREAM_CUTS")) {
        cuts.clear();
        for (const char* q = e; *q;) {
            char* endp = nullptr;
            const long v = strtol(q, &endp, 10);
            if (endp == q) break;
            if (v > 0 && v < 1000 && (cuts.empty() || (uint32_t)v > cuts.back()) && cuts.size() + 1 < (size_t)PO_MAX_PIECES) cuts.push_back((uint32_t)v);
            q = *endp ? endp + 1 : endp;
        }
    }
    std::vector<uint32_t> b{0};
    const uint64_t total = h->words[0].size();
    for (uint32_t c : cuts) {
        const uint64_t target = total * c / 1000;
        uint32_t lo = 0, hi = n / 2;
        while (lo < hi) {
            const uint32_t mid = (lo + hi) / 2;
            if (h->woff[2 * (size_t)mid] >= target) hi = mid; else lo = mid + 1;
        }
        if (2 * lo > b.back() && 2 * lo < n) b.push_back(2 * lo);
    }
    b.push_back(n);
    return b;
}

po_status stream_begin(po_handle* h, const std::vector<uint32_t>& bounds) {
    const uint32_t n = (uint32_t)h->len.size();
    const uint32_t P = (uint32_t)bounds.size() - 1;
    bool generate = false;
    if (!h->up_stream) HIP_TRY(h, hipStreamCreateWithFlags(&h->up_stream, hipStreamNonBlocking));
    for (uint32_t k = 0; k < P; ++k)
        if (!h->ev_piece[k]) HIP_TRY(h, hipEventCreate(&h->ev_piece[k]));
    auto queue_piece = [&](uint32_t k) -> po_status {
        uint64_t* dw = h->d_words.as<uint64_t>();
        const uint64_t wb = bounds[k] < n ? h->woff[bounds[k]] : h->words[0].size();
        const uint64_t we = bounds[k + 1] < n ? h->woff[bounds[k + 1]] : h->words[0].size();
        if (we > wb) {
            HIP_TRY(h, hipMemcpyAsync(dw + wb, h->words[0].data() + wb, (we - wb) * 8, hipMemcpyHostToDevice, h->up_stream));
            h->upload_bytes += (we - wb) * 8;
        }
        HIP_TRY(h, hipEventRecord(h->ev_piece[k], h->up_stream));
        return PO_OK;
    };
    PO_TRY(upload_meta(h, &generate));
    if (!generate) return fail(h, PO_ERR_INVALID, "streamed step on reads that are not (x, reverse complement of x) pairs");
    uint64_t* dw = h->d_words.as<uint64_t>();
    if (h->poison >= 0) {
        HIP_TRY(h, hipEventRecord(h->ev_up1, h->stream));
        HIP_TRY(h, hipStreamWaitEvent(h->up_stream, h->ev_up1, 0));
    }
    HIP_TRY(h, hipEventRecord(h->ev_up0, h->up_stream));
    PO_TRY(queue_piece(0));
    if (P > 1) {
        const uint32_t r0 = h->st_early_index ? 0u : bounds[1];
        if (h->st_lead > 2) {
            note_lead_words(h);
            PO_TRY(ensure(h, h->d_first, (size_t)n * LEAD_WORDS * 8));
            HIP_TRY(h, hipMemcpyAsync(h->d_first.as<uint64_t>() + (size_t)LEAD_WORDS * r0, h->lead_words.data() + (size_t)LEAD_WORDS * r0,
                                      (size_t)(n - r0) * LEAD_WORDS * 8, hipMemcpyHostToDevice, h->stream));
            h->upload_bytes += (size_t)(n - r0) * LEAD_WORDS * 8;
            hipLaunchKernelGGL(po::k_scatter_lead, dim3(cdiv((uint64_t)(n - r0) * LEAD_WORDS, 256)), dim3(256), 0, h->stream, dw,
                               h->d_woff.as<uint64_t>(), h->d_len.as<uint32_t>(), h->d_first.as<uint64_t>(), LEAD_WORDS, r0, n);
        } else {
            note_first_words(h);
            PO_TRY(ensure(h, h->d_first, (size_t)n * 16));
            HIP_TRY(h, hipMemcpyAsync(h->d_first.as<uint64_t>() + 2 * (size_t)r0, h->first_words.data() + 2 * (size_t)r0,
                                      (size_t)(n - r0) * 16, hipMemcpyHostToDevice, h->stream));
            h->upload_bytes += (size_t)(n - r0) * 16;
            hipLaunchKernelGGL(po::k_scatter_first, dim3(cdiv(n - r0, 256)), dim3(256), 0, h->stream, dw, h->d_woff.as<uint64_t>(),
                               h->d_first.as<ulonglong2>(), r0, n);
        }
        HIP_TRY(h, hipGetLastError());
        if (!h->ev_first) HIP_TRY(h, hipEventCreateWithFlags(&h->ev_first, hipEventDisableTiming));
        HIP_TRY(h, hipEventRecord(h->ev_first, h->stream));
        HIP_TRY(h, hipStreamWaitEvent(h->up_stream, h->ev_first, 0));
    }
    for (uint32_t k = 1; k < P; ++k) PO_TRY(queue_piece(k));
    HIP_TRY(h, hipEventRecord(h->ev_up1, h->up_stream));
    if (!h->rc_stream) HIP_TRY(h, hipStreamCreateWithFlags(&h->rc_stream, hipStreamNonBlocking));
    if (!h->ev_meta) HIP_TRY(h, hipEventCreateWithFlags(&h->ev_meta, hipEventDisableTiming));
    HIP_TRY(h, hipEventRecord(h->ev_meta, h->stream));
    HIP_TRY(h, hipStreamWaitEvent(h->rc_stream, h->ev_meta, 0));
    for (uint32_t k = 0; k < P; ++k) {
        if (!h->ev_rc[k]) HIP_TRY(h, hipEventCreateWithFlags(&h->ev_rc[k], hipEventDisableTiming));
        HIP_TRY(h, hipStreamWaitEvent(h->rc_stream, h->ev_piece[k], 0));
        const uint32_t p0 = bounds[k] / 2, p1 = bounds[k + 1] / 2;
        if (p1 > p0)
            hipLaunchKernelGGL(po::k_revcomp_store, dim3(cdiv((uint64_t)(p1 - p0) * 64, 256)), dim3(256), 0, h->rc_stream, dw,
                               h->d_woff.as<uint64_t>(), h->d_len.as<uint32_t>(), p0, p1,
                               h->n_exc_uploaded ? h->d_exc_off.as<uint32_t>() : nullptr, h->d_exc_pos.as<uint32_t>());
        HIP_TRY(h, hipGetLastError());
        HIP_TRY(h, hipEventRecord(h->ev_rc[k], h->rc_stream));
    }
    h->st_defer_cap = std::max<uint32_t>(1u << 16, h->defer_need + h->defer_need / 2);
    if (const char* e = getenv("PHASM_DEFER_CAP")) h->st_defer_cap = (uint32_t)std::max(1, atoi(e));
    PO_TRY(ensure(h, h->d_defer, (size_t)h->st_defer_cap * sizeof(po::Cand) + 16));
    if (!getenv("PHASM_DEFER_CAP")) h->st_defer_cap = (uint32_t)std::min<size_t>((h->d_defer.cap - 16) / sizeof(po::Cand), 0xFFFFFF00u);
    HIP_TRY(h, hipMemsetAsync(h->d_defer.as<char>() + (size_t)h->st_defer_cap * sizeof(po::Cand), 0, 16, h->stream));
    h->paired = true;
    ++h->upload_gen;
    h->dirty = false;
    return PO_OK;
}

po_status overlaps_streamed(po_handle* h, uint32_t min_length, HostRows& R, po_stats& sum, bool* overflow) {
    *overflow = false;
    const uint32_t n = (uint32_t)h->len.size();
    const std::vector<uint32_t> bounds = stream_bounds(h);
    const uint32_t P = (uint32_t)bounds.size() - 1;
    const bool trace = getenv("PHASM_STREAM_TRACE") != nullptr;
    const auto t_start = std::chrono::steady_clock::now();
    auto since = [&]() { return std::chrono::duration<double, std::milli>(std::chrono::steady_clock::now() - t_start).count(); };
    std::vector<uint32_t> sig(bounds);
    sig.push_back(min_length);
    sig.push_back((uint32_t)(h->total_bases & 0xFFFFFFFFu));
    h->st_pred_valid = h->st_pred_valid && sig == h->st_pred_sig;
    uint64_t new_pred[PO_MAX_PIECES] = {};
    h->st_selfclean = false;
    h->st_early_index = P > 1 && h->poison < 0 && !getenv("PHASM_NO_INDEX_REUSE") && !getenv("PHASM_LATE_INDEX");
    h->st_lead = index_flavour(h, min_length ? min_length : 1, true, LEAD_WORDS, OverlapSwitches()).ww >= 4 && !getenv("PHASM_STREAM_LEAD2") ? LEAD_WORDS : 2u;
    PO_TRY(stream_begin(h, bounds));
    auto piece_args = [&](uint32_t k) {
        OverlapArgs a{min_length, k, P};
        a.streamed = true;
        a.r_begin = bounds[k];
        a.r_end = bounds[k + 1];
        return a;
    };
    if (trace) std::fprintf(stderr, "[stream] %u pieces queued at %.3f ms\n", P, since());
    if (h->st_early_index) {
        po_result part;
        part.h = h;
        OverlapArgs a = piece_args(0);
        a.idx_only = true;
        const po_status ist = run_overlaps<2>(h, a, &part);
        part.d_rows.release();
        if (ist != PO_OK) {
            (void)hipStreamSynchronize(h->stream);
            (void)hipStreamSynchronize(h->up_stream);
            (void)hipStreamSynchronize(h->rc_stream);
            h->dirty = true;
            return ist;
        }
    }
    uint64_t* dw = h->d_words.as<uint64_t>();
    po_status st = PO_OK;
    auto completed = [&](uint32_t k, const po_stats& S, uint64_t nk) -> po_status {
        add_stats(sum, S);
        new_pred[k] = S.n_candidates;
        const double seen = (double)bounds[k + 1] / (double)n;
        if (h->chunk_compact[k]) PO_TRY(append_home(h, R, h->chunk_rows[k], S.n_verified, nk, k, P, seen * seen));
        else PO_TRY(append_rows(h, R, h->chunk_rows[k], nk, k, P, seen * seen));
        if (trace) {
            float up = 0;
            (void)hipEventElapsedTime(&up, h->ev_up0, h->ev_piece[k]);
            std::fprintf(stderr, "[stream] piece %u reads [%u, %u): landed %.3f ms after the first copy started, rows counted at %.3f ms (device %.3f ms: scan %.3f verify %.3f), %llu rows (%.1f MB) queued for home\n",
                         k, bounds[k], bounds[k + 1], up, since(), S.ms_total, S.ms_scan_count + S.ms_scan_fill, S.ms_verify,
                         (unsigned long long)nk, nk * 24e-6);
        }
        return PO_OK;
    };
    h->st_pend.valid = false;
    bool tail_gave_up = false;
    h->st_harvest = [&]() -> po_status {
        const uint32_t k = h->st_pend.k;
        bool needs_classic = false;
        const uint64_t nk = finish_piece(h, &needs_classic);
        if (needs_classic) {
            tail_gave_up = true;
            return PO_OK;
        }
        return completed(k, h->st_pend.S, nk);
    };
    if (getenv("PHASM_STREAM_SYNC")) h->st_harvest = nullptr;
    for (uint32_t k = 0; k < P && st == PO_OK; ++k) {
        if (hipStreamWaitEvent(h->stream, h->ev_rc[k], 0) != hipSuccess) { st = fail(h, PO_ERR_HIP, "hipStreamWaitEvent"); break; }
        OverlapArgs a = piece_args(k);
        {
            const double mine = (double)bounds[k + 1] * bounds[k + 1] - (double)bounds[k] * bounds[k];
            for (uint32_t j = k + 1; j < P; ++j)
                a.ws_scale = std::max(a.ws_scale, ((double)bounds[j + 1] * bounds[j + 1] - (double)bounds[j] * bounds[j]) / mine * 1.1);
        }
        h->ev = h->ev_sets[k & 1];
        uint64_t nk = 0;
        st = run_chunk(h, a, &nk);
        if (st != PO_OK || tail_gave_up) break;
        if (h->st_pend.valid && h->st_pend.k == k) continue;
        if (h->st_pend.valid) {
            if (hipStreamSynchronize(h->stream) != hipSuccess) { st = fail(h, PO_ERR_HIP, "stream"); break; }
            st = h->st_harvest();
            if (st != PO_OK) break;
        }
        st = completed(k, h->stats, nk);
    }
    if (st == PO_OK && h->st_pend.valid && !tail_gave_up) {
        if (hipStreamSynchronize(h->stream) != hipSuccess) st = fail(h, PO_ERR_HIP, "stream");
        else st = h->st_harvest();
    }
    h->st_harvest = nullptr;
    h->st_pend.valid = false;
    h->ev = h->ev_sets[0];
    if (st == PO_OK && tail_gave_up) {
        (void)hipStreamSynchronize(h->stream);
        (void)hipStreamSynchronize(h->up_stream);
        (void)hipStreamSynchronize(h->rc_stream);
        h->dirty = true;
        h->st_tail_gave_up = true;
        h->st_pred_valid = false;
        *overflow = true;
        return PO_OK;
    }
    if (st != PO_OK) {
        (void)hipStreamSynchronize(h->up_stream);
        (void)hipStreamSynchronize(h->rc_stream);
        h->dirty = true;
        h->st_pred_valid = false;
        return st;
    }
    h->st_pred_sig = sig;
    std::memcpy(h->st_pred_cand, new_pred, sizeof(new_pred));
    h->st_pred_valid = true;
    float ms = 0;
    (void)hipEventSynchronize(h->ev_up1);
    (void)hipEventElapsedTime(&ms, h->ev_up0, h->ev_up1);
    h->stats.ms_upload = ms;
    HIP_TRY(h, hipMemcpyAsync(h->pinned + 40, h->d_defer.as<char>() + (size_t)h->st_defer_cap * sizeof(po::Cand), 8,
                              hipMemcpyDeviceToHost, h->stream));
    HIP_TRY(h, hipStreamSynchronize(h->stream));
    const uint32_t n_def = (uint32_t)h->pinned[40];
    h->defer_need = n_def;
    if (n_def > h->st_defer_cap) {
        *overflow = true;
        return PO_OK;
    }
    if (n_def) {
        hipStream_t s = h->stream;
        po::Cand* list = h->d_defer.as<po::Cand>();
        PO_TRY(ensure(h, h->d_rowcnt, (size_t)n_def));
        PO_TRY(ensure(h, h->d_row_off, ((size_t)n_def + 1) * 4));
        HIP_TRY(h, hipEventRecord(h->ev[EV_START], s));
        hipLaunchKernelGGL(po::k_verify_flat, dim3(cdiv((uint64_t)n_def * 64, 256)), dim3(256), 0, s, dw, h->d_woff.as<uint64_t>(),
                           h->d_len.as<uint32_t>(), list, n_def, h->n_exc_uploaded ? h->d_exc_off.as<uint32_t>() : nullptr,
                           h->d_exc_pos.as<uint32_t>(), h->d_exc_byte.as<uint8_t>());
        hipLaunchKernelGGL(po::k_deferred_rowcnt, dim3(cdiv(n_def, 256)), dim3(256), 0, s, list, n_def, 1u, h->d_rowcnt.as<uint8_t>());
        HIP_TRY(h, hipGetLastError());
        PO_TRY(prefix_sum<uint8_t>(h, h->d_rowcnt.as<uint8_t>(), n_def, h->d_row_off.as<uint32_t>(), &h->pinned[2]));
        HIP_TRY(h, hipStreamSynchronize(s));
        const uint64_t n_rows = h->pinned[2];
        if (n_rows) {
            PO_TRY(ensure(h, h->chunk_rows[P], n_rows * sizeof(po_row)));
            unsigned long long* scalars = h->d_scalars.as<unsigned long long>();
            HIP_TRY(h, hipMemsetAsync(scalars + 4, 0, 32, s));
            hipLaunchKernelGGL(po::k_emit_cands, dim3(std::min<uint32_t>(cdiv(n_def, 256), (uint32_t)h->n_cu * 16)), dim3(256), 0, s,
                               list, h->d_rowcnt.as<uint8_t>(), h->d_row_off.as<uint32_t>(), n_def, h->d_len.as<uint32_t>(),
                               h->chunk_rows[P].as<po::Row>(), 2u, 1u, scalars + 4);
            HIP_TRY(h, hipGetLastError());
            HIP_TRY(h, hipMemcpyAsync(h->pinned + 4, scalars + 4, 4 * sizeof(uint64_t), hipMemcpyDeviceToHost, s));
            HIP_TRY(h, hipEventRecord(h->ev[EV_EMIT], s));
            HIP_TRY(h, hipStreamSynchronize(s));
            float ms_def = 0;
            (void)hipEventElapsedTime(&ms_def, h->ev[EV_START], h->ev[EV_EMIT]);
            sum.n_verified += h->pinned[4];
            sum.sum_overlap_bases += h->pinned[5];
            sum.verify_bytes_algo += h->pinned[6];
            sum.verify_bytes_exec += h->pinned[7];
            sum.n_rows += n_rows;
            sum.ms_verify += ms_def;
            sum.ms_total += ms_def;
            PO_TRY(append_rows(h, R, h->chunk_rows[P], n_rows, P, P + 1));
        }
    }
    (void)n;
    if (trace) {
        std::fprintf(stderr, "[stream] deferred list settled at %.3f ms (%u candidates)\n", since(), n_def);
        (void)hipStreamSynchronize(h->copy_stream);
        std::fprintf(stderr, "[stream] last row home at %.3f ms\n", since());
    }
    return PO_OK;
}

}
}

po_status po_overlaps_to_host(po_handle* h, uint32_t min_length, po_result** out) {
    if (!h || !out) return PO_ERR_INVALID;
    *out = nullptr;
    if (h->segments_only) return fail(h, PO_ERR_INVALID, "this handle holds GFA segments without sequences: nothing to overlap");
    uint32_t n_chunks = (h->len.size() >= 8192 && h->total_bases >= (64ull << 20)) ? 4u : 1u;
    if (const char* e = getenv("PHASM_HOST_CHUNKS")) n_chunks = (uint32_t)std::max(1, std::min(4, atoi(e)));
    po_result* r = new (std::nothrow) po_result();
    if (!r) return fail(h, PO_ERR_NOMEM, "out of host memory");
    r->h = h;
    po_status st = PO_OK;
    HostRows R;
    po_stats sum = {};
    bool streamed = false, overflowed = false;
    float ms_upload = 0;
    try {
        st = init_device(h);
        if (st == PO_OK && !h->copy_stream && hipStreamCreateWithFlags(&h->copy_stream, hipStreamNonBlocking) != hipSuccess)
            st = fail(h, PO_ERR_HIP, "cannot create the copy stream");
        if (st == PO_OK && h->spare_host.p) {
            R.hb = h->spare_host;
            h->spare_host = HostBuf();
        }
        if (st == PO_OK) {
            (void)home_begin(h);
            h->home_last_bytes = 0;
        }
        if (st == PO_OK && stream_eligible(h, min_length)) {
            bool overflow = false;
            st = overlaps_streamed(h, min_length, R, sum, &overflow);
            ms_upload = h->stats.ms_upload;
            if (st == PO_OK && !overflow) {
                streamed = true;
            } else if (st == PO_OK) {
                overflowed = true;
                home_wait(h);
                if (h->home_on) {
                    home::g_pool->sum_l.store(0);
                    home::g_pool->sum_b.store(0);
                    home::g_pool->sum_e.store(0);
                }
                if (hipStreamSynchronize(h->copy_stream) != hipSuccess) st = fail(h, PO_ERR_HIP, "copy stream");
                R.total = 0;
                sum = po_stats();
            }
        }
        if (st == PO_OK && !streamed) st = upload(h);
        for (uint32_t k = 0; k < n_chunks && st == PO_OK && !streamed; ++k) {
            uint64_t nk = 0;
            st = run_chunk(h, OverlapArgs{min_length, k, n_chunks}, &nk);
            if (st != PO_OK) break;
            add_stats(sum, h->stats);
            st = h->chunk_compact[k] ? append_home(h, R, h->chunk_rows[k], h->stats.n_verified, nk, k, n_chunks)
                                     : append_rows(h, R, h->chunk_rows[k], nk, k, n_chunks);
        }
    } catch (const std::bad_alloc&) {
        st = fail(h, PO_ERR_NOMEM, "out of host memory in po_overlaps_to_host");
    }
    h->st_harvest = nullptr;
    h->st_pend.valid = false;
    h->ev = h->ev_sets[0];
    if (h->dev_ready) (void)hipStreamSynchronize(h->stream);
    if (h->up_stream) (void)hipStreamSynchronize(h->up_stream);
    if (h->rc_stream) (void)hipStreamSynchronize(h->rc_stream);
    if (h->copy_stream && hipStreamSynchronize(h->copy_stream) != hipSuccess && st == PO_OK) st = fail(h, PO_ERR_HIP, "row copy device->host");
    {
        const int herr = home_end(h, &sum);
        if (herr && st == PO_OK)
            st = fail(h, PO_ERR_HIP, herr == 1 ? "internal: the host's row count of a piece differs from the device's"
                                     : herr == 2 ? "internal: a verified-candidate record names a read the handle does not hold"
                                                 : "the event behind a device->host copy of records failed");
    }
    if (st != PO_OK) {
        R.hb.release();
        delete r;
        return st;
    }
    po_stats& S = h->stats;
    S.n_candidates = sum.n_candidates;
    S.n_verified = sum.n_verified;
    S.n_rows = sum.n_rows;
    S.sum_overlap_bases = sum.sum_overlap_bases;
    S.verify_bytes_algo = sum.verify_bytes_algo;
    S.verify_bytes_exec = sum.verify_bytes_exec;
    S.n_tiles = sum.n_tiles;
    S.shard_bases = sum.shard_bases;
    S.ms_index = sum.ms_index;
    S.ms_scan_count = sum.ms_scan_count;
    S.ms_scan_fill = sum.ms_scan_fill;
    S.ms_verify = sum.ms_verify;
    S.ms_select = sum.ms_select;
    S.ms_emit = sum.ms_emit;
    S.ms_total = sum.ms_total;
    S.ms_scan_probe = sum.ms_scan_probe;
    S.ms_verify_kernel = sum.ms_verify_kernel;
    S.fused_tail = sum.fused_tail;
// ... 851 lines not shown
    return PO_OK;
}

po_status po_relevant_copy(po_result* out, uint32_t* cur_aligning, uint32_t* rel_reads, int32_t* overlap_max, uint32_t* aln_off,
                           uint32_t* aln_b, int32_t* aln_a0, int32_t* aln_a1, uint32_t* b_reads) {
    if (!out) return PO_ERR_INVALID;
    if (out->special != 2) return fail(out->h, PO_ERR_INVALID, "po_relevant_copy needs the result of po_phase_relevant");
    auto give = [](void* dst, const void* src, size_t n) {
        if (dst && n) std::memcpy(dst, src, n * 4);
    };
    give(cur_aligning, out->rv_ca.data(), out->rv_ca.size());
    give(rel_reads, out->rv_rel.data(), out->rv_rel.size());
    give(overlap_max, out->rv_om.data(), out->rv_om.size());
    if (aln_off && out->rv_alnoff.empty()) aln_off[0] = 0;
    give(aln_off, out->rv_alnoff.data(), out->rv_alnoff.size());
    give(aln_b, out->rv_alnb.data(), out->rv_alnb.size());
    give(aln_a0, out->rv_a0.data(), out->rv_a0.size());
    give(aln_a1, out->rv_a1.data(), out->rv_a1.size());
    give(b_reads, out->rv_b.data(), out->rv_b.size());
    return PO_OK;
}

po_status po_get_relevant_stats(const po_handle* h, po_relevant_stats* out) { return get_stats(h, &po_handle::rvstats, out); }

po_status po_spell(po_handle* h, const po_spell_input* in, po_result** out) {
    if (!h) return PO_ERR_INVALID;
    if (!out) return fail(h, PO_ERR_INVALID, "po_spell: no room for the result");
    *out = nullptr;
    if (!in) return fail(h, PO_ERR_INVALID, "po_spell: no input");
    if (in->n_pieces >= 0xFFFFFFFFull || in->n_seqs >= 0xFFFFFFFFull)
        return fail(h, PO_ERR_CAPACITY, "po_spell: more than 2^32 - 2 pieces or sequences in one call");
    uint64_t n_bytes = 0, n_patched = 0;
    const std::string said = spell_check(h, *in, &n_bytes, &n_patched);
    if (!said.empty()) return fail(h, PO_ERR_INVALID, said);
    if (n_bytes > SPELL_MAX_BYTES)
        return fail(h, PO_ERR_CAPACITY, "po_spell: " + std::to_string(n_bytes) + " bytes in one call, at most 2^32 - 16");
    PO_TRY(init_device(h));
    return new_edge_result(h, "po_spell", out, [&](po_result* r) { return run_spell(h, *in, n_bytes, n_patched, r); });
}

po_status po_spell_sizes(const po_result* out, uint64_t* n_seqs, uint64_t* n_bytes) {
    if (!out || !n_seqs || !n_bytes) return PO_ERR_INVALID;
    if (out->special != 3) return fail(out->h, PO_ERR_INVALID, "po_spell_sizes needs the result of po_spell");
    *n_seqs = out->sp_off.size() - 1;
    *n_bytes = out->sp_off.back();
    return PO_OK;
}

po_status po_spell_copy(po_result* out, uint64_t* seq_byte_off, uint8_t* bytes, uint64_t cap) {
    if (!out) return PO_ERR_INVALID;
    po_handle* h = out->h;
    if (out->special != 3) return fail(h, PO_ERR_INVALID, "po_spell_copy needs the result of po_spell");
    if (seq_byte_off) std::memcpy(seq_byte_off, out->sp_off.data(), out->sp_off.size() * 8);
    const uint64_t n_give = bytes ? std::min<uint64_t>(cap, out->sp_off.back()) : 0;
    if (!n_give) return PO_OK;
    constexpr uint64_t STEP = 64ull << 20;
    return guarded_run(h, "po_spell_copy", [&] {
        PO_TRY(ensure_host(h, h->scratch_host, (size_t)std::min(n_give, STEP)));
        for (uint64_t at = 0; at < n_give; at += STEP) {
            const size_t k = (size_t)std::min(STEP, n_give - at);
            HIP_TRY(h, hipMemcpyAsync(h->scratch_host.p, out->d_rows.as<char>() + at, k, hipMemcpyDeviceToHost, h->stream));
            HIP_TRY(h, hipStreamSynchronize(h->stream));
            std::memcpy(bytes + at, h->scratch_host.p, k);
        }
        return PO_OK;
    });
}

po_status po_get_spell_stats(const po_handle* h, po_spell_stats* out) { return get_stats(h, &po_handle::spstats, out); }

po_status po_result_merged_paths(po_result* r, uint64_t* n_paths, uint64_t* n_members, uint64_t* offsets_out, uint64_t cap_paths,
                                 uint32_t* members_out, int32_t* prefix_out, uint64_t cap_members, int64_t* lengths_out) {
    if (!r || !n_paths || !n_members) return PO_ERR_INVALID;
    *n_paths = *n_members = 0;
    po_handle* h = r->h;
    if (!h) return PO_ERR_INVALID;
    if (!r->merged) return fail(h, PO_ERR_INVALID, "po_result_merged_paths needs a po_layout_merge result");
    const uint64_t K = r->n_merged, m = r->n_members;
    *n_paths = K;
    *n_members = m;
    try {
        (void)hipSetDevice(h->device);
        HIP_TRY(h, hipStreamSynchronize(h->stream));
        if (offsets_out && cap_paths >= K) {
            std::vector<uint32_t> off(K);
            if (K) HIP_TRY(h, hipMemcpy(off.data(), r->d_moff.p, K * 4, hipMemcpyDeviceToHost));
            for (uint64_t k = 0; k < K; ++k) offsets_out[k] = off[k];
            offsets_out[K] = m;
        }
        if (lengths_out && cap_paths >= K && K) HIP_TRY(h, hipMemcpy(lengths_out, r->d_mlen.p, K * 8, hipMemcpyDeviceToHost));
        if (members_out && cap_members >= m && m) HIP_TRY(h, hipMemcpy(members_out, r->d_member.p, m * 4, hipMemcpyDeviceToHost));
        if (prefix_out && cap_members >= m && m) HIP_TRY(h, hipMemcpy(prefix_out, r->d_prefix.p, m * 4, hipMemcpyDeviceToHost));
    } catch (const std::bad_alloc&) {
        return fail(h, PO_ERR_NOMEM, "out of host memory in po_result_merged_paths");
    }
    return PO_OK;
}

po_status po_result_node_order(po_result* r, uint32_t* nodes_out, uint64_t cap, uint64_t* n_out) {
    if (!r || !n_out || (!nodes_out && cap)) return PO_ERR_INVALID;
    *n_out = 0;
    po_handle* h = r->h;
    if (!h) return PO_ERR_INVALID;
    if (!r->kind_edges || !r->d_nrank.p) return fail(h, PO_ERR_INVALID, "po_result_node_order needs an edge result");
    const size_t n_nodes = h->len.size() + (r->merged ? (size_t)r->n_merged : 0);
    try {
        std::vector<unsigned long long> rank(n_nodes);
        (void)hipSetDevice(h->device);
        HIP_TRY(h, hipStreamSynchronize(h->stream));
        if (n_nodes) HIP_TRY(h, hipMemcpy(rank.data(), r->d_nrank.p, n_nodes * 8, hipMemcpyDeviceToHost));
        std::vector<std::pair<unsigned long long, uint32_t>> order;
        for (size_t i = 0; i < n_nodes; ++i)
            if (rank[i] != po::NODE_NO_RANK) order.emplace_back(rank[i], (uint32_t)i);
        std::sort(order.begin(), order.end());
        *n_out = order.size();
        for (size_t i = 0; i < order.size() && i < cap; ++i) nodes_out[i] = order[i].second;
    } catch (const std::bad_alloc&) {
        return fail(h, PO_ERR_NOMEM, "out of host memory in po_result_node_order");
    }
    return PO_OK;
}

uint64_t po_debug_host_ranges(uint64_t* out, uint64_t cap_entries) {
    std::lock_guard<std::mutex> lock(g_pin_mu);
    const uint64_t n = std::min<uint64_t>(cap_entries, g_pins.size());
    for (uint64_t i = 0; out && i < n; ++i) {
        out[3 * i] = g_pins[i].base;
        out[3 * i + 1] = g_pins[i].bytes;
        out[3 * i + 2] = g_pins[i].kind;
    }
    return g_pins.size();
}

uint64_t po_debug_store_words(const po_handle* h, int store, const uint64_t** words) {
    if (!h || store < 0 || store > 1) return 0;
    if (words) *words = h->words[store].data();
    return h->words[store].size();
}

int po_debug_expand_records(const po_cand* records, uint64_t n, const uint32_t* lengths, uint32_t n_reads, uint32_t paired,
                            po_row* rows_out, uint64_t n_rows_expected) {
    home::Pool* P = home::pool();
    if (!P) return -1;
    std::lock_guard<std::mutex> call(P->call_mu);
    home::begin(P, lengths, n_reads, false);
    home::Job j;
    j.rec = records;
    j.n_rec = n;
    j.out = rows_out;
    j.n_rows = n_rows_expected;
    j.paired = paired ? 1u : 0u;
    home::submit(P, j);
    home::wait_all(P);
    return P->error.load();
}

int po_debug_expand_packed(const uint64_t* records, uint64_t n, uint32_t sh_b, uint32_t sh_p, const uint32_t* lengths, uint32_t n_reads,
                           uint32_t paired, po_row* rows_out, uint64_t n_rows_expected) {
    if (!sh_b || sh_p < sh_b || sh_p >= 62) return -2;
    home::Pool* P = home::pool();
    if (!P) return -1;
    std::lock_guard<std::mutex> call(P->call_mu);
    home::begin(P, lengths, n_reads, false);
    home::Job j;
    j.rec = records;
    j.sh_b = sh_b;
    j.sh_p = sh_p;
    j.n_rec = n;
    j.out = rows_out;
    j.n_rows = n_rows_expected;
    j.paired = paired ? 1u : 0u;
    home::submit(P, j);
    home::wait_all(P);
    return P->error.load();
}

static int g_fault_fd = 2;
static struct sigaction g_fault_prev[2];
static void fault_handler(int sig, siginfo_t* si, void* ctx) {
    char line[128];
    const int n = std::snprintf(line, sizeof(line), "[phasm] signal %d at address %p (code %d); native stack of the faulting thread:\n", sig,
                                si ? si->si_addr : nullptr, si ? si->si_code : 0);
    if (n > 0) (void)!::write(g_fault_fd, line, (size_t)n);
    void* frames[64];
    const int k = backtrace(frames, 64);
    backtrace_symbols_fd(frames, k, g_fault_fd);
    const struct sigaction& prev = g_fault_prev[sig == SIGBUS ? 1 : 0];
    if ((prev.sa_flags & SA_SIGINFO) && prev.sa_sigaction) {
        prev.sa_sigaction(sig, si, ctx);
        return;
    }
    if (prev.sa_handler != SIG_DFL && prev.sa_handler != SIG_IGN && prev.sa_handler) {
        prev.sa_handler(sig);
        return;
    }
    signal(sig, SIG_DFL);
    raise(sig);
}

int po_debug_fault_backtrace(int fd) {
    g_fault_fd = fd;
    struct sigaction sa;
    std::memset(&sa, 0, sizeof(sa));
    sa.sa_sigaction = fault_handler;
    sa.sa_flags = SA_SIGINFO | SA_NODEFER;
    sigemptyset(&sa.sa_mask);
    void* warm[4];
    (void)backtrace(warm, 4);
    return (sigaction(SIGSEGV, &sa, &g_fault_prev[0]) == 0 && sigaction(SIGBUS, &sa, &g_fault_prev[1]) == 0) ? 0 : -1;
}

int po_debug_pointer_info(const void* p, int32_t* hip_type, int32_t* hsa_type, uint64_t* base, uint64_t* bytes) {
    if (hip_type) *hip_type = -1;
    if (hsa_type) *hsa_type = -1;
    if (base) *base = 0;
    if (bytes) *bytes = 0;
    if (!p) return 0;
    int known = 0;
    {
        hipPointerAttribute_t at;
        std::memset(&at, 0, sizeof(at));
        const hipError_t e = hipPointerGetAttributes(&at, p);
        if (e == hipSuccess) {
            if (hip_type) *hip_type = (int32_t)at.type;
            if (at.type != hipMemoryTypeUnregistered) known = 1;
        } else {
            (void)hipGetLastError();
        }
    }
    {
        struct PtrInfo {
            uint32_t size;
            uint32_t type;
            void* agentBaseAddress;
            void* hostBaseAddress;
            size_t sizeInBytes;
            void* userData;
            uint64_t agentOwner;
            uint32_t global_flags;
        };
        using Fn = int (*)(const void*, PtrInfo*, void* (*)(size_t), uint32_t*, void**);
        static Fn fn = reinterpret_cast<Fn>(dlsym(RTLD_DEFAULT, "hsa_amd_pointer_info"));
        if (fn) {
            PtrInfo info;
            std::memset(&info, 0, sizeof(info));
            info.size = sizeof(info);
            if (fn(p, &info, nullptr, nullptr, nullptr) == 0) {
                if (hsa_type) *hsa_type = (int32_t)info.type;
                if (info.type != 0) {
                    known = 1;
                    if (base) *base = (uint64_t)(uintptr_t)(info.hostBaseAddress ? info.hostBaseAddress : info.agentBaseAddress);
                    if (bytes) *bytes = info.sizeInBytes;
                }
            }
        }
    }
    return known;
}

po_status po_get_stats(const po_handle* h, po_stats* out) {
    if (!h || !out) return PO_ERR_INVALID;
    *out = h->stats;
    return PO_OK;
}

const char* po_last_error(const po_handle* h) { return h ? h->err.c_str() : "null handle"; }

}
```

### phasm_amd/csrc/kernels.hip.h

```cpp
#pragma once
#include <hip/hip_runtime.h>
#include <stdint.h>

namespace po {

using u32x4 = __attribute__((ext_vector_type(4))) uint32_t;

constexpr uint32_t NO_SELFREP = 0xFFFFFFFFu;
constexpr uint64_t KEY_EMPTY = ~0ull;
constexpr int WAVE = 64;

#ifndef PO_VER_PAD
#define PO_VER_PAD 0
#endif
#ifndef PO_SCAN_PAD
#define PO_SCAN_PAD 0
#endif
template <int N>
__device__ __forceinline__ void valu_pad(uint32_t& r, uint32_t c) {
#pragma unroll
    for (int i = 0; i < N; ++i) asm volatile("v_xor_b32 %0, %0, %1" : "+v"(r) : "v"(c));
}

struct CandGuard {
// ... 1808 lines not shown
                          const uint8_t* __restrict__ flag, const uint32_t* __restrict__ flag_off, uint32_t n_cand,
                          Cand* __restrict__ out, uint32_t cap) {
    uint32_t i = blockIdx.x * blockDim.x + threadIdx.x;
    if (i >= n_cand || flag[i] == 0) return;
    const uint32_t o = flag_off[i];
    if (o < cap) out[o] = Cand{cand_a[i], cand_p[i], cand_b[i], type[i]};
}

__global__ void k_flag(const uint8_t* __restrict__ rowcnt, uint32_t n, uint8_t* __restrict__ flag) {
    uint32_t i = blockIdx.x * blockDim.x + threadIdx.x;
    if (i < n) flag[i] = rowcnt[i] != 0;
}

__global__ void k_cand_rowcnt(const Cand* __restrict__ cands, uint32_t n, uint32_t n_reads, uint32_t paired,
                              uint8_t* __restrict__ rowcnt, uint32_t* __restrict__ n_bad) {
    uint32_t i = blockIdx.x * blockDim.x + threadIdx.x;
    if (i >= n) return;
    const Cand c = cands[i];
    if ((c.a | c.p | c.b | c.type) == 0) {
        rowcnt[i] = 0;
        return;
    }
    if (c.a >= n_reads || c.b >= n_reads || c.a == c.b || c.type == 0 || c.type > 3) {
        rowcnt[i] = 0;
        atomicAdd(n_bad, 1u);
        return;
    }
    rowcnt[i] = (uint8_t)rows_of(c.type, c.a, c.b, paired);
}

__global__ __launch_bounds__(256) void k_emit_cands(const Cand* __restrict__ cands, const uint8_t* __restrict__ rowcnt,
                                                    const uint32_t* __restrict__ row_off, uint32_t n,
                                                    const uint32_t* __restrict__ len, Row* __restrict__ rows,
                                                    uint32_t bits, uint32_t paired,
                                                    unsigned long long* __restrict__ counters) {
    uint64_t nver = 0, suml = 0, sumb = 0, sume = 0;
    for (uint32_t i = blockIdx.x * blockDim.x + threadIdx.x; i < n; i += gridDim.x * blockDim.x) {
        if (rowcnt[i] == 0) continue;
        const Cand c = cands[i];
        nver += 1;
        write_rows(rows, row_off[i], c.type, c.a, c.p, c.b, len[c.a], len[c.b], bits, paired, suml, sumb, sume);
    }
    flush_counters(nver, suml, sumb, sume, counters);
}

__global__ __launch_bounds__(256) void k_paired_check(const uint64_t* __restrict__ words, const uint64_t* __restrict__ woff,
                                                      const uint32_t* __restrict__ len, uint32_t n_pairs,
                                                      const uint8_t* __restrict__ pair_state,
                                                      uint32_t* __restrict__ n_bad) {
    const uint32_t pair = (blockIdx.x * blockDim.x + threadIdx.x) >> 6;
    if (pair >= n_pairs) return;
    const uint32_t lane = lane_id();
    const uint32_t L = len[2 * pair];
    bool bad = false;
    const uint32_t hs = pair_state ? pair_state[pair] : 0u;
    if (hs != 0) {
        bad = hs == 2;
    } else if (len[2 * pair + 1] != L) {
        bad = true;
    } else {
        const uint64_t* __restrict__ R = words + woff[2 * pair];
        const uint64_t* __restrict__ S = words + woff[2 * pair + 1];
        const uint32_t nw = (L + 31) / 32;
        for (uint32_t w = lane; w < nw && !bad; w += WAVE) {
            const int64_t o = (int64_t)L - 32 * (int64_t)w - 32;
            uint64_t x;
            uint32_t valid = 32;
            if (o >= 0) {
                x = funnel(R[o >> 5], R[(o >> 5) + 1], (uint32_t)(o & 31) * 2);
            } else {
                valid = (uint32_t)(32 + o);
                x = R[0] << ((uint32_t)(-o) * 2);
            }
            uint64_t y = __brevll(x);
            y = ((y >> 1) & 0x5555555555555555ull) | ((y & 0x5555555555555555ull) << 1);
            y = ~y;
            const uint64_t mask = valid >= 32 ? ~0ull : ((1ull << (valid * 2)) - 1ull);
            bad = ((y ^ S[w]) & mask) != 0;
        }
    }
    if (__any(bad) && lane == 0) atomicAdd(n_bad, 1u);
}

__global__ __launch_bounds__(256) void k_revcomp_store(uint64_t* __restrict__ words, const uint64_t* __restrict__ woff,
                                                       const uint32_t* __restrict__ len, uint32_t pair0, uint32_t n_pairs,
                                                       const uint32_t* __restrict__ exc_off, const uint32_t* __restrict__ exc_pos) {
    const uint32_t pair = pair0 + ((blockIdx.x * blockDim.x + threadIdx.x) >> 6);
    if (pair >= n_pairs) return;
    const uint32_t e0 = exc_off ? exc_off[2 * pair + 1] : 0u, e1 = exc_off ? exc_off[2 * pair + 2] : 0u;
    const uint32_t lane = lane_id();
    const uint32_t L = len[2 * pair];
    const uint64_t* __restrict__ R = words + woff[2 * pair];
    uint64_t* __restrict__ S = words + woff[2 * pair + 1];
    const uint32_t nw = (L + 31) / 32;
    const uint32_t last = nw + (uint32_t)((woff[2 * pair + 1] + nw + 1) & 1ull);
    for (uint32_t w = lane; w <= last; w += WAVE) {
        uint64_t out = 0;
        if (w < nw) {
            const int64_t o = (int64_t)L - 32 * (int64_t)w - 32;
            uint64_t x;
            uint32_t valid = 32;
            if (o >= 0) {
                x = funnel(R[o >> 5], R[(o >> 5) + 1], (uint32_t)(o & 31) * 2);
            } else {
                valid = (uint32_t)(32 + o);
                x = R[0] << ((uint32_t)(-o) * 2);
            }
            uint64_t y = __brevll(x);
            y = ((y >> 1) & 0x5555555555555555ull) | ((y & 0x5555555555555555ull) << 1);
            y = ~y;
            out = valid >= 32 ? y : (y & ((1ull << (valid * 2)) - 1ull));
            for (uint32_t e = e0; e < e1; ++e) {
                const uint32_t pos = exc_pos[e];
                if ((pos >> 5) == w) out &= ~(3ull << ((pos & 31u) * 2u));
            }
        }
        S[w] = out;
    }
}

__global__ void k_scatter_first(uint64_t* __restrict__ words, const uint64_t* __restrict__ woff,
                                const ulonglong2* __restrict__ first, uint32_t r0, uint32_t n) {
    const uint32_t r = r0 + blockIdx.x * blockDim.x + threadIdx.x;
    if (r >= n) return;
    const ulonglong2 f = first[r];
    *reinterpret_cast<ulonglong2*>(words + woff[r]) = f;
}

__global__ void k_scatter_lead(uint64_t* __restrict__ words, const uint64_t* __restrict__ woff, const uint32_t* __restrict__ len,
                               const uint64_t* __restrict__ lead, uint32_t nw, uint32_t r0, uint32_t n) {
    const uint64_t t = (uint64_t)blockIdx.x * blockDim.x + threadIdx.x;
    const uint64_t r = r0 + t / nw;
    const uint32_t k = (uint32_t)(t % nw);
    if (r >= n) return;
    const uint32_t own = (len[r] + 31u) / 32u + 1u;
    if (k < own) words[woff[r] + k] = lead[r * nw + k];
}

__global__ void k_defer_split(const uint32_t* __restrict__ cand_a, const uint32_t* __restrict__ cand_p,
                              const uint32_t* __restrict__ cand_b, uint32_t n_cand, uint32_t b_limit, Cand* __restrict__ out,
                              uint32_t cap, uint32_t* __restrict__ counter, const CandGuard G) {
    const uint32_t i = blockIdx.x * blockDim.x + threadIdx.x;
    if (G.n_dev) {
        if (G.overflow()) return;
        n_cand = (uint32_t)*G.n_dev;
    }
    if (i >= n_cand) return;
    const uint32_t b = cand_b[i];
    if (b < b_limit) return;
    const uint32_t k = atomicAdd(counter, 1u);
    if (k < cap) out[k] = Cand{cand_a[i], cand_p[i], b, 0u};
}

__global__ __launch_bounds__(256) void k_verify_flat(const uint64_t* __restrict__ words, const uint64_t* __restrict__ woff,
                                                     const uint32_t* __restrict__ len, Cand* __restrict__ cands, uint32_t n,
                                                     const uint32_t* __restrict__ exc_off, const uint32_t* __restrict__ exc_pos,
                                                     const uint8_t* __restrict__ exc_byte) {
    const uint32_t i = (blockIdx.x * blockDim.x + threadIdx.x) >> 6;
    if (i >= n) return;
    const uint32_t lane = lane_id();
    const Cand c = cands[i];
    const uint32_t la = len[c.a], lb = len[c.b];
    bool bad = c.p > la || la - c.p < lb || c.a == c.b || (c.a & 1u);
    if (!bad) {
        const uint64_t* __restrict__ A = words + woff[c.a] + (c.p >> 5);
        const uint64_t* __restrict__ B = words + woff[c.b];
        const uint32_t sh = (c.p & 31u) * 2u, nw = (lb + 31u) >> 5;
        for (uint32_t w = lane; w < nw; w += WAVE) {
            uint64_t d = funnel(A[w], A[w + 1], sh) ^ B[w];
            if (w == nw - 1 && (lb & 31u)) d &= (1ull << ((lb & 31u) * 2u)) - 1ull;
            bad |= d != 0;
        }
    }
    bool any_bad = __any(bad);
    if (lane == 0 && !any_bad && exc_off && !exceptions_equal(exc_off, exc_pos, exc_byte, c.a, c.p, c.b, lb)) any_bad = true;
    if (lane == 0) cands[i].type = any_bad ? 0u : 2u;
}

__global__ void k_deferred_rowcnt(const Cand* __restrict__ cands, uint32_t n, uint32_t paired, uint8_t* __restrict__ rowcnt) {
    const uint32_t i = blockIdx.x * blockDim.x + threadIdx.x;
    if (i >= n) return;
    const Cand c = cands[i];
    rowcnt[i] = c.type ? (uint8_t)rows_of(c.type, c.a, c.b, paired) : (uint8_t)0;
}

constexpr int PS_BLOCK = 256;
constexpr int PS_ITEMS = 16;
constexpr int PS_TILE = PS_BLOCK * PS_ITEMS;

template <typename T>
__global__ __launch_bounds__(PS_BLOCK) void k_ps_reduce(const T* __restrict__ in, uint64_t n, uint64_t* __restrict__ block_sums) {
    __shared__ uint64_t s_part[PS_BLOCK / WAVE];
    const uint64_t base = (uint64_t)blockIdx.x * PS_TILE;
    uint64_t acc = 0;
    const uint64_t first = base + (uint64_t)threadIdx.x * PS_ITEMS;
    if (first + PS_ITEMS <= n && (reinterpret_cast<uintptr_t>(in + first) & 15u) == 0) {
        const u32x4* src = reinterpret_cast<const u32x4*>(in + first);
#pragma unroll
        for (int k = 0; k < (int)(PS_ITEMS * sizeof(T) / 16); ++k) {
            const u32x4 q = src[k];
            if constexpr (sizeof(T) == 1) {
                const uint32_t d[4] = {q.x, q.y, q.z, q.w};
#pragma unroll
                for (int j = 0; j < 4; ++j) acc += (d[j] & 0xFFu) + ((d[j] >> 8) & 0xFFu) + ((d[j] >> 16) & 0xFFu) + (d[j] >> 24);
            } else {
                acc += (uint64_t)q.x + q.y + q.z + q.w;
            }
        }
    } else {
        for (int k = 0; k < PS_ITEMS; ++k)
            if (first + k < n) acc += in[first + k];
    }
    acc = wave_sum64(acc);
    if (lane_id() == 0) s_part[threadIdx.x >> 6] = acc;
    __syncthreads();
    if (threadIdx.x == 0) {
        uint64_t s = 0;
        for (int w = 0; w < PS_BLOCK / WAVE; ++w) s += s_part[w];
        block_sums[blockIdx.x] = s;
    }
}

__global__ __launch_bounds__(1024) void k_ps_spine(uint64_t* __restrict__ block_sums, uint32_t nblocks, uint64_t* __restrict__ total,
                                                  uint64_t* __restrict__ total_host, const uint64_t* __restrict__ also_src = nullptr,
                                                  uint64_t* __restrict__ also_host = nullptr) {
    __shared__ uint64_t s_wave[1024 / WAVE];
    const uint32_t per = (nblocks + 1023) / 1024;
    const uint32_t lo = min(threadIdx.x * per, nblocks);
    const uint32_t hi = min(lo + per, nblocks);
    uint64_t acc = 0;
    for (uint32_t i = lo; i < hi; ++i) acc += block_sums[i];
    uint64_t incl = acc;
#pragma unroll
    for (int d = 1; d < WAVE; d <<= 1) {
        const uint64_t up = __shfl_up(incl, d, WAVE);
        if (lane_id() >= (uint32_t)d) incl += up;
    }
    if (lane_id() == WAVE - 1) s_wave[threadIdx.x >> 6] = incl;
    __syncthreads();
    uint64_t run = incl - acc;
    for (uint32_t w = 0; w < (threadIdx.x >> 6); ++w) run += s_wave[w];
    if (threadIdx.x == 1023) {
        *total = run + acc;
        *total_host = run + acc;
        if (also_src) *also_host = *also_src;
    }
    for (uint32_t i = lo; i < hi; ++i) {
        const uint64_t v = block_sums[i];
        block_sums[i] = run;
        run += v;
    }
}

constexpr uint32_t PS_SMALL_MAX = 1u << 13;
__global__ __launch_bounds__(1024) void k_ps_small(uint32_t* __restrict__ in, const uint32_t* __restrict__ extra, uint32_t n,
                                                  uint32_t* __restrict__ out, uint64_t* __restrict__ total,
                                                  uint64_t* __restrict__ total_host, const uint64_t* __restrict__ also_src,
                                                  uint64_t* __restrict__ also_host) {
    __shared__ uint64_t s_wave[1024 / WAVE];
    const uint32_t per = (n + 1023) / 1024;
    const uint32_t lo = min(threadIdx.x * per, n);
    const uint32_t hi = min(lo + per, n);
    uint64_t acc = 0;
    for (uint32_t i = lo; i < hi; ++i) {
        uint32_t v = in[i];
        if (extra && extra[i]) {
            v += extra[i];
            in[i] = v;
        }
        acc += v;
    }
    uint64_t incl = acc;
#pragma unroll
    for (int d = 1; d < WAVE; d <<= 1) {
        const uint64_t up = __shfl_up(incl, d, WAVE);
        if (lane_id() >= (uint32_t)d) incl += up;
    }
    if (lane_id() == WAVE - 1) s_wave[threadIdx.x >> 6] = incl;
    __syncthreads();
    uint64_t run = incl - acc;
    for (uint32_t w = 0; w < (threadIdx.x >> 6); ++w) run += s_wave[w];
    if (threadIdx.x == 1023) {
        *total = run + acc;
        *total_host = run + acc;
        out[n] = (uint32_t)(run + acc);
        if (also_src) *also_host = *also_src;
    }
    for (uint32_t i = lo; i < hi; ++i) {
        out[i] = (uint32_t)run;
        run += in[i];
    }
}

template <typename T>
__global__ __launch_bounds__(PS_BLOCK) void k_ps_down(const T* __restrict__ in, uint64_t n, const uint64_t* __restrict__ block_sums,
                                                      uint32_t* __restrict__ out) {
    static_assert(PS_ITEMS == 16, "vector paths assume 16 items per thread");
    __shared__ uint32_t s_wave[PS_BLOCK / WAVE];
    const uint64_t base = (uint64_t)blockIdx.x * PS_TILE + (uint64_t)threadIdx.x * PS_ITEMS;
    const bool full = base + PS_ITEMS <= n;
    uint32_t v[PS_ITEMS];
    if (full && (reinterpret_cast<uintptr_t>(in + base) & 15u) == 0) {
        if constexpr (sizeof(T) == 1) {
            const u32x4 q = *reinterpret_cast<const u32x4*>(in + base);
            const uint32_t w[4] = {q.x, q.y, q.z, q.w};
#pragma unroll
            for (int k = 0; k < PS_ITEMS; ++k) v[k] = (w[k >> 2] >> (8 * (k & 3))) & 0xFFu;
        } else {
#pragma unroll
            for (int g = 0; g < 4; ++g) {
                const u32x4 q = *reinterpret_cast<const u32x4*>(in + base + 4 * g);
                v[4 * g] = q.x;
                v[4 * g + 1] = q.y;
                v[4 * g + 2] = q.z;
                v[4 * g + 3] = q.w;
            }
        }
    } else {
#pragma unroll
        for (int k = 0; k < PS_ITEMS; ++k) {
            const uint64_t i = base + k;
            v[k] = i < n ? (uint32_t)in[i] : 0u;
        }
    }
    uint32_t acc = 0;
#pragma unroll
    for (int k = 0; k < PS_ITEMS; ++k) acc += v[k];
    const uint32_t incl = wave_incl_scan(acc);
    if (lane_id() == WAVE - 1) s_wave[threadIdx.x >> 6] = incl;
// ... 477 lines not shown
```

Measured before the change: 1.561 billion.

## Vectorise host row expansion, spin-wait home workers, and queue deferred verification on device

Moves host-side record expansion into a new header with an AVX2 path that counts and writes rows using streaming stores. Worker threads now spin while a call is open instead of waiting on a condition variable, which cuts wake-up latency at the cost of burning CPU cycles. In the streaming pipeline the deferred candidate list is verified and compacted on the GPU after the last piece, with its records sent home through pinned memory, so a later synchronous verification round trip is avoided. The change also adds a debug sums query and a scalar fallback environment switch.

Result: slower. 1.544 billion (-1.1%).

```diff
diff --git a/include/phasm_overlap.h b/include/phasm_overlap.h
--- a/include/phasm_overlap.h
+++ b/include/phasm_overlap.h
@@ -593,6 +593,7 @@
                             po_row* rows_out, uint64_t n_rows_expected);
 int po_debug_expand_packed(const uint64_t* records, uint64_t n, uint32_t sh_b, uint32_t sh_p, const uint32_t* lengths, uint32_t n_reads,
                            uint32_t paired, po_row* rows_out, uint64_t n_rows_expected);
+int po_debug_expand_sums(uint64_t out[4]);
 int po_debug_fault_backtrace(int fd);
 int po_debug_pointer_info(const void* p, int32_t* hip_type, int32_t* hsa_type, uint64_t* base, uint64_t* bytes);
 
diff --git a/phasm_amd/_lib.py b/phasm_amd/_lib.py
--- a/phasm_amd/_lib.py
+++ b/phasm_amd/_lib.py
@@ -413,6 +413,7 @@
                                               ctypes.c_uint32, ctypes.c_void_p, ctypes.c_uint64]),
     ("po_debug_expand_records", ctypes.c_int, [ctypes.c_void_p, ctypes.c_uint64, ctypes.c_void_p, ctypes.c_uint32, ctypes.c_uint32,
                                                ctypes.c_void_p, ctypes.c_uint64]),
+    ("po_debug_expand_sums", ctypes.c_int, [ctypes.POINTER(ctypes.c_uint64)]),
     ("po_debug_host_ranges", ctypes.c_uint64, [ctypes.POINTER(ctypes.c_uint64), ctypes.c_uint64]),
     ("po_debug_pointer_info", ctypes.c_int, [ctypes.c_void_p, ctypes.POINTER(ctypes.c_int32), ctypes.POINTER(ctypes.c_int32),
                                              ctypes.POINTER(ctypes.c_uint64), ctypes.POINTER(ctypes.c_uint64)]),
diff --git a/phasm_amd/csrc/c_api.hip b/phasm_amd/csrc/c_api.hip
--- a/phasm_amd/csrc/c_api.hip
+++ b/phasm_amd/csrc/c_api.hip
@@ -46,6 +46,7 @@
 #include "phase.hip.h"
 #include "relevant.hip.h"
 #include "spell.hip.h"
+#include "home_expand.h"
 
 namespace {
 
@@ -147,6 +148,8 @@
 }
 
 constexpr int PO_MAX_PIECES = 16;
+constexpr uint32_t DEFER_RECORDS_LIMIT = 1u << 18;
+constexpr uint32_t DEFER_ZONE = 40;
 
 struct RegHeader {
     size_t bytes;
@@ -660,17 +663,18 @@
 
 namespace home {
 
+using namespace home_expand;
 constexpr uint32_t CHUNK = 4096;
-
-struct Job {
-    const void* rec = nullptr;
-    uint32_t sh_b = 0, sh_p = 0;
+static_assert(sizeof(Rec) == sizeof(po::Cand) && offsetof(Rec, a) == offsetof(po::Cand, a) && offsetof(Rec, p) == offsetof(po::Cand, p) &&
+                  offsetof(Rec, b) == offsetof(po::Cand, b) && offsetof(Rec, type) == offsetof(po::Cand, type),
+              "home_expand::Rec is po::Cand");
+
+struct Job : Recs {
     uint64_t n_rec = 0;
     po_row* out = nullptr;
     uint64_t n_rows = 0;
     const volatile uint32_t* flag = nullptr;
     uint32_t want = 0;
-    uint32_t paired = 0, bits = 2;
 };
 
 struct Pool {
@@ -684,9 +688,11 @@
     std::atomic<int> error{0};
     const uint32_t* len = nullptr;
     uint32_t n_reads = 0;
+    int level = 0;
     std::atomic<uint64_t> sum_l{0}, sum_b{0}, sum_e{0};
     Job cur;
-    uint64_t job_seq = 0;
+    std::atomic<uint64_t> job_seq{0};
+    std::atomic<int> open{0};
     uint32_t n_chunks = 0;
     std::vector<uint64_t> chunk_off;
     std::atomic<uint32_t> next_count{0}, done_count{0}, next_write{0}, done_write{0};
@@ -716,68 +722,13 @@
     }
 }
 
-inline po::Cand load_rec(const Job& j, uint64_t i) {
-    if (!j.sh_b) return static_cast<const po::Cand*>(j.rec)[i];
-    return po::unpack_record(static_cast<const uint64_t*>(j.rec)[i], j.sh_b, j.sh_p);
-}
-
-inline uint32_t rows_of_rec(const po::Cand& c, uint32_t paired) {
-    if (!paired) return (c.type & 1u) + ((c.type >> 1) & 1u);
-    return ((c.type & 1u) ? (c.a == (c.b ^ 1u) ? 1u : 2u) : 0u) + ((c.type & 2u) ? 2u : 0u);
-}
-
-inline void put_row(uint64_t*& o, uint32_t a, uint32_t b, uint32_t astart, uint32_t aend, uint32_t bend) {
-    __builtin_nontemporal_store((uint64_t)a | ((uint64_t)b << 32), o);
-    __builtin_nontemporal_store((uint64_t)astart | ((uint64_t)aend << 32), o + 1);
-    __builtin_nontemporal_store((uint64_t)bend << 32, o + 2);
-    o += 3;
-}
-
-bool expand_records(Pool& P, uint64_t lo, uint64_t hi, po_row* out) {
-    uint64_t* o = reinterpret_cast<uint64_t*>(out);
-    const Job& job = P.cur;
-    const uint32_t* len = P.len;
-    const uint32_t paired = job.paired, n_reads = P.n_reads, bits = job.bits;
-    auto pb = [bits](uint32_t l) -> uint64_t { return bits == 8u ? l : (l >> 2) + ((l & 3u) != 0u); };
-    uint64_t sl = 0, sb = 0, se = 0;
-    for (uint64_t i = lo; i < hi; ++i) {
-        const po::Cand c = load_rec(job, i);
-        if (c.a >= n_reads || c.b >= n_reads) return false;
-        const uint32_t la = len[c.a], lb = len[c.b];
-        se += 2 * pb((c.type & 1u) ? la - c.p : lb);
-        if (c.type & 1u) {
-            const uint32_t l = la - c.p;
-            const bool twin = paired && c.a != (c.b ^ 1u);
-            put_row(o, c.a, c.b, c.p, la, l);
-            if (twin) put_row(o, c.b ^ 1u, c.a ^ 1u, lb - l, lb, l);
-            const uint64_t k = twin ? 2 : 1;
-            sl += k * l;
-            sb += k * 2 * pb(l);
-        }
-        if (c.type & 2u) {
-            put_row(o, c.a, c.b, c.p, c.p + lb, lb);
-            if (paired) put_row(o, c.a ^ 1u, c.b ^ 1u, la - c.p - lb, la - c.p, lb);
-            const uint64_t k = paired ? 2 : 1;
-            sl += k * lb;
-            sb += k * 2 * pb(lb);
-        }
-    }
-    P.sum_l.fetch_add(sl, std::memory_order_relaxed);
-    P.sum_b.fetch_add(sb, std::memory_order_relaxed);
-    P.sum_e.fetch_add(se, std::memory_order_relaxed);
-    return true;
-}
-
 void run_phases(Pool& P, bool lead) {
     const uint32_t nc = P.n_chunks;
     for (;;) {
         const uint32_t c = P.next_count.fetch_add(1, std::memory_order_relaxed);
         if (c >= nc) break;
         const uint64_t lo = (uint64_t)c * CHUNK, hi = std::min<uint64_t>(P.cur.n_rec, lo + CHUNK);
-        uint64_t n = 0;
-        const uint32_t paired = P.cur.paired;
-        for (uint64_t i = lo; i < hi; ++i) n += rows_of_rec(load_rec(P.cur, i), paired);
-        P.chunk_off[c + 1] = n;
+        P.chunk_off[c + 1] = count_chunk(P.cur, lo, hi, P.level);
         P.done_count.fetch_add(1, std::memory_order_release);
     }
     if (lead) {
@@ -794,7 +745,11 @@
         const uint32_t c = P.next_write.fetch_add(1, std::memory_order_relaxed);
         if (c >= nc) break;
         const uint64_t lo = (uint64_t)c * CHUNK, hi = std::min<uint64_t>(P.cur.n_rec, lo + CHUNK);
-        if (!expand_records(P, lo, hi, P.cur.out + P.chunk_off[c])) P.error.store(2);
+        Sums sums;
+        if (!write_chunk(P.cur, P.len, P.n_reads, lo, hi, P.cur.out + P.chunk_off[c], sums, P.level)) P.error.store(2);
+        P.sum_l.fetch_add(sums.l, std::memory_order_relaxed);
+        P.sum_b.fetch_add(sums.b, std::memory_order_relaxed);
+        P.sum_e.fetch_add(sums.e, std::memory_order_relaxed);
 #if defined(__x86_64__)
         __builtin_ia32_sfence();
 #endif
@@ -806,14 +761,19 @@
     Pool& P = *Pp;
     uint64_t seen = 0;
     for (;;) {
-        {
-            std::unique_lock<std::mutex> lock(P.mu);
-            P.cv_job.wait(lock, [&] { return P.job_seq != seen; });
-            seen = P.job_seq;
-        }
-        P.inside.fetch_add(1, std::memory_order_acq_rel);
-        if (P.phase.load(std::memory_order_acquire) != 0) run_phases(P, false);
-        P.inside.fetch_sub(1, std::memory_order_release);
+        uint64_t seq;
+        while ((seq = P.job_seq.load(std::memory_order_seq_cst)) == seen) {
+            if (P.open.load(std::memory_order_acquire)) {
+                spin_until([&] { return P.job_seq.load(std::memory_order_acquire) != seen || !P.open.load(std::memory_order_acquire); });
+            } else {
+                std::unique_lock<std::mutex> lock(P.mu);
+                P.cv_job.wait(lock, [&] { return P.job_seq.load(std::memory_order_acquire) != seen || P.open.load(std::memory_order_acquire); });
+            }
+        }
+        seen = seq;
+        P.inside.fetch_add(1, std::memory_order_seq_cst);
+        if (P.phase.load(std::memory_order_seq_cst) != 0) run_phases(P, false);
+        P.inside.fetch_sub(1, std::memory_order_seq_cst);
     }
 }
 
@@ -832,7 +792,7 @@
         std::atomic_thread_fence(std::memory_order_acquire);
         const double t_ready = P.tracing ? std::chrono::duration<double, std::micro>(std::chrono::steady_clock::now() - P.t0).count() : 0.0;
         if (P.error.load() == 0 && j.n_rec) {
-            spin_until([&] { return P.inside.load(std::memory_order_acquire) == 0; });
+            spin_until([&] { return P.inside.load(std::memory_order_seq_cst) == 0; });
             P.cur = j;
             P.n_chunks = (uint32_t)((j.n_rec + CHUNK - 1) / CHUNK);
             if (P.chunk_off.size() < (size_t)P.n_chunks + 1) P.chunk_off.resize((size_t)P.n_chunks + 1);
@@ -840,17 +800,12 @@
             P.done_count.store(0);
             P.next_write.store(0);
             P.done_write.store(0);
-            P.phase.store(1, std::memory_order_release);
-            {
-                std::lock_guard<std::mutex> lock(P.mu);
-                ++P.job_seq;
-            }
-            P.cv_job.notify_all();
+            P.phase.store(1, std::memory_order_seq_cst);
+            P.job_seq.fetch_add(1, std::memory_order_seq_cst);
             run_phases(P, true);
             if (P.phase.load() == 2)
                 spin_until([&] { return P.done_write.load(std::memory_order_acquire) >= P.n_chunks; });
-            P.phase.store(0, std::memory_order_release);
-            std::atomic_thread_fence(std::memory_order_seq_cst);
+            P.phase.store(0, std::memory_order_seq_cst);
         }
         if (P.tracing)
             P.trace.push_back({t_ready, std::chrono::duration<double, std::micro>(std::chrono::steady_clock::now() - P.t0).count(), (double)j.n_rows});
@@ -885,6 +840,8 @@
 void begin(Pool* P, const uint32_t* len, uint32_t n_reads, bool tracing) {
     if (const char* e = getenv("PHASM_HOME_SPIN")) g_spin_limit.store((uint32_t)std::max(0, atoi(e)));
     else g_spin_limit.store(4096);
+    const char* sc = getenv("PHASM_HOME_SCALAR");
+    P->level = (sc && atoi(sc) != 0) ? 0 : vector_level();
     P->len = len;
     P->n_reads = n_reads;
     P->error.store(0);
@@ -896,6 +853,15 @@
     P->tracing = tracing;
     P->trace.clear();
     P->t0 = std::chrono::steady_clock::now();
+    {
+        std::lock_guard<std::mutex> lock(P->mu);
+        P->open.store(1, std::memory_order_release);
+    }
+    P->cv_job.notify_all();
+}
+
+void end(Pool* P) {
+    P->open.store(0, std::memory_order_release);
 }
 
 void submit(Pool* P, const Job& j) {
@@ -1002,7 +968,7 @@
             (const void*)po::k_verify_a<2, false, true, true>, (const void*)po::k_verify_a<2, false, true, false>,
             (const void*)po::k_verify_a<2, true, true, false>, (const void*)po::k_select_local, (const void*)po::k_tile_rows<true>,
             (const void*)po::k_tile_rows<false>, (const void*)po::k_tail, (const void*)po::k_tail_cands, (const void*)po::k_select,
-            (const void*)po::k_emit, (const void*)po::k_verify_flat, (const void*)po::k_deferred_rowcnt, (const void*)po::k_emit_cands,
+            (const void*)po::k_emit, (const void*)po::k_verify_flat, (const void*)po::k_verify_flat_dev, (const void*)po::k_defer_records, (const void*)po::k_deferred_rowcnt, (const void*)po::k_emit_cands,
             (const void*)po::k_wide_insert<2, 1>, (const void*)po::k_wide_insert<2, 16>, (const void*)po::k_wide_chain_fill<2, 1>,
             (const void*)po::k_wide_chain_fill<2, 16>, (const void*)po::k_wide_finalize<2, 1>, (const void*)po::k_wide_finalize<2, 16>,
             (const void*)po::k_chain_sort_short<uint64_t>, (const void*)po::k_chain_sort_long<uint64_t>,
@@ -5469,6 +5435,7 @@
             std::fprintf(stderr, "[home] piece %zu: records home at %.3f ms, %.0f rows written at %.3f ms (since the call set the pool up)\n", i,
                          P->trace[i][0] * 1e-3, P->trace[i][2], P->trace[i][1] * 1e-3);
     h->home_on = false;
+    home::end(P);
     P->call_mu.unlock();
     return err;
 }
@@ -5499,6 +5466,7 @@
     const size_t elem = h->home_sh_b ? sizeof(uint64_t) : sizeof(po::Cand);
     const size_t bytes = (size_t)n_rec * elem;
     constexpr uint64_t N_EV = 32;
+    static_assert(96 + N_EV <= 1024 / sizeof(uint64_t), "the flag words lie inside the 1 KB landing zone");
     if (h->home_used + bytes > h->home_stage.cap || (h->home_seq && h->home_seq % N_EV == 0)) {
         home_wait(h);
         if (hipStreamSynchronize(h->copy_stream) != hipSuccess) return fail(h, PO_ERR_HIP, "copy stream");
@@ -5767,6 +5735,8 @@
         return PO_OK;
     };
     h->st_pend.valid = false;
+    const bool defer_records = h->home_on && P > 1;
+    bool defer_queued = false;
     bool tail_gave_up = false;
     h->st_harvest = [&]() -> po_status {
         const uint32_t k = h->st_pend.k;
@@ -5788,6 +5758,21 @@
                 a.ws_scale = std::max(a.ws_scale, ((double)bounds[j + 1] * bounds[j + 1] - (double)bounds[j] * bounds[j]) / mine * 1.1);
         }
         h->ev = h->ev_sets[k & 1];
+        if (defer_records && k == P - 1) {
+            const uint32_t room = std::min<uint32_t>(h->st_defer_cap, DEFER_RECORDS_LIMIT);
+            st = ensure(h, h->chunk_rows[P], (size_t)room * sizeof(po::Cand));
+            if (st != PO_OK) break;
+            const uint32_t* n_dev = h->d_defer.as<uint32_t>() + (size_t)h->st_defer_cap * 4;
+            const uint32_t blocks = std::min<uint32_t>(std::max<uint32_t>(cdiv(h->defer_need, 4), (uint32_t)h->n_cu), 1u << 16);
+            hipLaunchKernelGGL(po::k_verify_flat_dev, dim3(blocks), dim3(256), 0, h->stream, dw, h->d_woff.as<uint64_t>(), h->d_len.as<uint32_t>(),
+                               h->d_defer.as<po::Cand>(), n_dev, h->st_defer_cap, DEFER_RECORDS_LIMIT,
+                               h->n_exc_uploaded ? h->d_exc_off.as<uint32_t>() : nullptr, h->d_exc_pos.as<uint32_t>(), h->d_exc_byte.as<uint8_t>());
+            hipLaunchKernelGGL(po::k_defer_records, dim3(1), dim3(po::DEFER_RECORDS_BLOCK), 0, h->stream, h->d_defer.as<po::Cand>(), n_dev,
+                               h->st_defer_cap, DEFER_RECORDS_LIMIT, h->chunk_rows[P].as<po::Cand>(), h->home_sh_b, h->home_sh_p,
+                               h->pinned_dev + DEFER_ZONE);
+            if (hipGetLastError() != hipSuccess || hipEventRecord(h->ev_first, h->stream) != hipSuccess) { st = fail(h, PO_ERR_HIP, "deferred list"); break; }
+            defer_queued = true;
+        }
         uint64_t nk = 0;
         st = run_chunk(h, a, &nk);
         if (st != PO_OK || tail_gave_up) break;
@@ -5830,6 +5815,29 @@
     (void)hipEventSynchronize(h->ev_up1);
     (void)hipEventElapsedTime(&ms, h->ev_up0, h->ev_up1);
     h->stats.ms_upload = ms;
+    if (defer_queued) {
+        HIP_TRY(h, hipEventSynchronize(h->ev_first));
+        const uint64_t n_def64 = h->pinned[DEFER_ZONE], n_rec = h->pinned[DEFER_ZONE + 1], n_rows = h->pinned[DEFER_ZONE + 2];
+        if (n_rec != ~0ull || n_def64 > h->st_defer_cap) {
+            h->defer_need = (uint32_t)n_def64;
+            if (n_def64 > h->st_defer_cap) {
+                *overflow = true;
+                return PO_OK;
+            }
+            if (n_rec) {
+                sum.n_verified += n_rec;
+                sum.n_rows += n_rows;
+                PO_TRY(append_home(h, R, h->chunk_rows[P], n_rec, n_rows, P, P + 1));
+            }
+            if (trace) {
+                std::fprintf(stderr, "[stream] deferred list: %llu candidates, %llu records queued for home at %.3f ms\n", (unsigned long long)n_def64,
+                             (unsigned long long)n_rec, since());
+                (void)hipStreamSynchronize(h->copy_stream);
+                std::fprintf(stderr, "[stream] last record home at %.3f ms\n", since());
+            }
+            return PO_OK;
+        }
+    }
     HIP_TRY(h, hipMemcpyAsync(h->pinned + 40, h->d_defer.as<char>() + (size_t)h->st_defer_cap * sizeof(po::Cand), 8,
                               hipMemcpyDeviceToHost, h->stream));
     HIP_TRY(h, hipStreamSynchronize(h->stream));
@@ -6987,6 +6995,7 @@
     j.paired = paired ? 1u : 0u;
     home::submit(P, j);
     home::wait_all(P);
+    home::end(P);
     return P->error.load();
 }
 
@@ -7007,7 +7016,19 @@
     j.paired = paired ? 1u : 0u;
     home::submit(P, j);
     home::wait_all(P);
+    home::end(P);
     return P->error.load();
+}
+
+int po_debug_expand_sums(uint64_t out[4]) {
+    home::Pool* P = home::pool();
+    if (!P) return -1;
+    std::lock_guard<std::mutex> call(P->call_mu);
+    out[0] = P->sum_l.load();
+    out[1] = P->sum_b.load();
+    out[2] = P->sum_e.load();
+    out[3] = (uint64_t)P->level;
+    return 0;
 }
 
 static int g_fault_fd = 2;
diff --git a/phasm_amd/csrc/home_expand.h b/phasm_amd/csrc/home_expand.h
--- /dev/null
+++ b/phasm_amd/csrc/home_expand.h
@@ -0,0 +1,274 @@
+#pragma once
+
+#include <cstddef>
+#include <cstdint>
+
+#if defined(__x86_64__)
+#include <immintrin.h>
+#define PHASM_HOME_AVX2 1
+#endif
+
+namespace home_expand {
+
+struct Rec {
+    uint32_t a, p, b, type;
+};
+
+struct Recs {
+    const void* rec = nullptr;
+    uint32_t sh_b = 0, sh_p = 0;
+    uint32_t paired = 0, bits = 2;
+};
+
+struct Sums {
+    uint64_t l = 0, b = 0, e = 0;
+};
+
+inline Rec unpack_rec(uint64_t v, uint32_t sh_b, uint32_t sh_p) {
+    const uint64_t mr = (1ull << sh_b) - 1ull;
+    return Rec{(uint32_t)(v & mr), (uint32_t)((v >> sh_p) & ((1ull << (62u - sh_p)) - 1ull)), (uint32_t)((v >> sh_b) & mr), (uint32_t)(v >> 62)};
+}
+
+inline Rec load_rec(const Recs& j, uint64_t i) {
+    if (!j.sh_b) return static_cast<const Rec*>(j.rec)[i];
+    return unpack_rec(static_cast<const uint64_t*>(j.rec)[i], j.sh_b, j.sh_p);
+}
+
+inline uint32_t rows_of_rec(const Rec& c, uint32_t paired) {
+    if (!paired) return (c.type & 1u) + ((c.type >> 1) & 1u);
+    return ((c.type & 1u) ? (c.a == (c.b ^ 1u) ? 1u : 2u) : 0u) + ((c.type & 2u) ? 2u : 0u);
+}
+
+inline void nt_store(uint64_t v, uint64_t* o) {
+#if defined(__x86_64__)
+    _mm_stream_si64(reinterpret_cast<long long*>(o), (long long)v);
+#else
+    *o = v;
+#endif
+}
+
+inline void put_row(uint64_t*& o, uint32_t a, uint32_t b, uint32_t astart, uint32_t aend, uint32_t bend) {
+    nt_store((uint64_t)a | ((uint64_t)b << 32), o);
+    nt_store((uint64_t)astart | ((uint64_t)aend << 32), o + 1);
+    nt_store((uint64_t)bend << 32, o + 2);
+    o += 3;
+}
+
+
+inline uint64_t count_chunk_scalar(const Recs& j, uint64_t lo, uint64_t hi) {
+    uint64_t n = 0;
+    for (uint64_t i = lo; i < hi; ++i) n += rows_of_rec(load_rec(j, i), j.paired);
+    return n;
+}
+
+inline bool write_span_scalar(const Recs& j, const uint32_t* len, uint32_t n_reads, uint64_t lo, uint64_t hi, uint64_t*& o, Sums& s) {
+    const uint32_t paired = j.paired, bits = j.bits;
+    auto pb = [bits](uint32_t l) -> uint64_t { return bits == 8u ? l : (l >> 2) + ((l & 3u) != 0u); };
+    uint64_t sl = 0, sb = 0, se = 0;
+    for (uint64_t i = lo; i < hi; ++i) {
+        const Rec c = load_rec(j, i);
+        if (c.a >= n_reads || c.b >= n_reads) return false;
+        const uint32_t la = len[c.a], lb = len[c.b];
+        se += 2 * pb((c.type & 1u) ? la - c.p : lb);
+        if (c.type & 1u) {
+            const uint32_t l = la - c.p;
+            const bool twin = paired && c.a != (c.b ^ 1u);
+            put_row(o, c.a, c.b, c.p, la, l);
+            if (twin) put_row(o, c.b ^ 1u, c.a ^ 1u, lb - l, lb, l);
+            const uint64_t k = twin ? 2 : 1;
+            sl += k * l;
+            sb += k * 2 * pb(l);
+        }
+        if (c.type & 2u) {
+            put_row(o, c.a, c.b, c.p, c.p + lb, lb);
+            if (paired) put_row(o, c.a ^ 1u, c.b ^ 1u, la - c.p - lb, la - c.p, lb);
+            const uint64_t k = paired ? 2 : 1;
+            sl += k * lb;
+            sb += k * 2 * pb(lb);
+        }
+    }
+    s.l += sl;
+    s.b += sb;
+    s.e += se;
+    return true;
+}
+
+inline bool write_chunk_scalar(const Recs& j, const uint32_t* len, uint32_t n_reads, uint64_t lo, uint64_t hi, void* out, Sums& s) {
+    uint64_t* o = static_cast<uint64_t*>(out);
+    Sums t;
+    if (!write_span_scalar(j, len, n_reads, lo, hi, o, t)) return false;
+    s.l += t.l;
+    s.b += t.b;
+    s.e += t.e;
+    return true;
+}
+
+#if defined(PHASM_HOME_AVX2)
+
+__attribute__((target("avx2"))) inline uint64_t count_chunk_avx2(const Recs& j, uint64_t lo, uint64_t hi) {
+    const uint64_t* r = static_cast<const uint64_t*>(j.rec);
+    const __m128i cb = _mm_cvtsi32_si128((int)j.sh_b);
+    const __m256i mr = _mm256_set1_epi64x((long long)((1ull << j.sh_b) - 1ull)), one = _mm256_set1_epi64x(1);
+    __m256i acc = _mm256_setzero_si256();
+    uint64_t i = lo;
+    if (j.paired) {
+        for (; i + 4 <= hi; i += 4) {
+            const __m256i v = _mm256_loadu_si256(reinterpret_cast<const __m256i*>(r + i));
+            const __m256i t1 = _mm256_and_si256(_mm256_srli_epi64(v, 62), one), t2 = _mm256_srli_epi64(v, 63);
+            const __m256i a = _mm256_and_si256(v, mr), b = _mm256_and_si256(_mm256_srl_epi64(v, cb), mr);
+            const __m256i self = _mm256_and_si256(_mm256_cmpeq_epi64(a, _mm256_xor_si256(b, one)), t1);
+            const __m256i t12 = _mm256_add_epi64(t1, t2);
+            acc = _mm256_add_epi64(acc, _mm256_sub_epi64(_mm256_add_epi64(t12, t12), self));
+        }
+    } else {
+        for (; i + 4 <= hi; i += 4) {
+            const __m256i v = _mm256_loadu_si256(reinterpret_cast<const __m256i*>(r + i));
+            acc = _mm256_add_epi64(acc, _mm256_add_epi64(_mm256_and_si256(_mm256_srli_epi64(v, 62), one), _mm256_srli_epi64(v, 63)));
+        }
+    }
+    alignas(32) uint64_t lanes[4];
+    _mm256_store_si256(reinterpret_cast<__m256i*>(lanes), acc);
+    return lanes[0] + lanes[1] + lanes[2] + lanes[3] + count_chunk_scalar(j, i, hi);
+}
+
+__attribute__((target("avx2"))) inline void quads_avx2(__m256i f0, __m256i f1, __m256i f2, __m256i f3, __m256i t[4]) {
+    const __m256i x0 = _mm256_unpacklo_epi32(f0, f1), x1 = _mm256_unpackhi_epi32(f0, f1);
+    const __m256i x2 = _mm256_unpacklo_epi32(f2, f3), x3 = _mm256_unpackhi_epi32(f2, f3);
+    t[0] = _mm256_unpacklo_epi64(x0, x2);
+    t[1] = _mm256_unpackhi_epi64(x0, x2);
+    t[2] = _mm256_unpacklo_epi64(x1, x3);
+    t[3] = _mm256_unpackhi_epi64(x1, x3);
+}
+
+__attribute__((target("avx2"))) inline __m256i narrow_avx2(__m256i lo, __m256i hi) {
+    const __m256i x = _mm256_castps_si256(_mm256_shuffle_ps(_mm256_castsi256_ps(lo), _mm256_castsi256_ps(hi), 0x88));
+    return _mm256_permute4x64_epi64(x, 0xD8);
+}
+
+__attribute__((target("avx2"))) inline void words_out_avx2(__m256i x, uint32_t n, uint64_t* o) {
+    alignas(32) uint64_t w[4];
+    _mm256_store_si256(reinterpret_cast<__m256i*>(w), x);
+    for (uint32_t k = 0; k < n; ++k) nt_store(w[k], o + k);
+}
+
+__attribute__((target("avx2"))) inline bool write_chunk_avx2(const Recs& j, const uint32_t* len, uint32_t n_reads, uint64_t lo, uint64_t hi, void* out,
+                                                             Sums& s) {
+    uint64_t* o = static_cast<uint64_t*>(out);
+    const uint64_t* r = static_cast<const uint64_t*>(j.rec);
+    Sums t;
+    if (!j.paired || !j.sh_b || n_reads > 0x80000000u || (reinterpret_cast<uintptr_t>(o) & 7u)) {
+        if (!write_span_scalar(j, len, n_reads, lo, hi, o, t)) return false;
+        s.l += t.l, s.b += t.b, s.e += t.e;
+        return true;
+    }
+    const __m128i cb = _mm_cvtsi32_si128((int)j.sh_b), cp = _mm_cvtsi32_si128((int)j.sh_p);
+    const __m256i mr = _mm256_set1_epi64x((long long)((1ull << j.sh_b) - 1ull));
+    const __m256i mp = _mm256_set1_epi64x((long long)((1ull << (62u - j.sh_p)) - 1ull));
+    const __m256i one64 = _mm256_set1_epi64x(1), one = _mm256_set1_epi32(1), zero = _mm256_setzero_si256();
+    const __m256i top = _mm256_set1_epi32((int)(n_reads - 1u)), low32 = _mm256_set1_epi64x(0xFFFFFFFFll), three = _mm256_set1_epi32(3);
+    const bool bytes = j.bits == 8u;
+    __m256i acc_l = zero, acc_pb = zero;
+    bool run = false;
+    uint32_t sh = 0;
+    __m256i rot = zero, mask = zero, carry = zero;
+    uint64_t i = lo;
+    for (; n_reads && i + 8 <= hi; i += 8) {
+        const __m256i v0 = _mm256_loadu_si256(reinterpret_cast<const __m256i*>(r + i));
+        const __m256i v1 = _mm256_loadu_si256(reinterpret_cast<const __m256i*>(r + i + 4));
+        const __m256i a0 = _mm256_and_si256(v0, mr), a1 = _mm256_and_si256(v1, mr);
+        const __m256i b0 = _mm256_and_si256(_mm256_srl_epi64(v0, cb), mr), b1 = _mm256_and_si256(_mm256_srl_epi64(v1, cb), mr);
+        const __m256i ty = _mm256_and_si256(_mm256_cmpeq_epi64(_mm256_srli_epi64(v0, 62), one64), _mm256_cmpeq_epi64(_mm256_srli_epi64(v1, 62), one64));
+        const __m256i self = _mm256_or_si256(_mm256_cmpeq_epi64(a0, _mm256_xor_si256(b0, one64)), _mm256_cmpeq_epi64(a1, _mm256_xor_si256(b1, one64)));
+        const __m256i a = narrow_avx2(a0, a1), b = narrow_avx2(b0, b1);
+        const __m256i ab = _mm256_max_epu32(a, b);
+        const __m256i known = _mm256_cmpeq_epi32(_mm256_min_epu32(ab, top), ab);
+        const bool fast = _mm256_movemask_epi8(ty) == -1 && _mm256_testz_si256(self, self) && _mm256_movemask_epi8(known) == -1;
+        if (!fast) {
+            if (run) words_out_avx2(carry, sh ? 4u - sh : 0u, o - (sh ? 4u - sh : 0u));
+            run = false;
+            if (!write_span_scalar(j, len, n_reads, i, i + 8, o, t)) return false;
+            continue;
+        }
+        const __m256i p = narrow_avx2(_mm256_and_si256(_mm256_srl_epi64(v0, cp), mp), _mm256_and_si256(_mm256_srl_epi64(v1, cp), mp));
+        const __m256i la = _mm256_i32gather_epi32(reinterpret_cast<const int*>(len), a, 4);
+        const __m256i lb = _mm256_i32gather_epi32(reinterpret_cast<const int*>(len), b, 4);
+        const __m256i l = _mm256_sub_epi32(la, p);
+        const __m256i pbl = bytes ? l : _mm256_add_epi32(_mm256_add_epi32(_mm256_srli_epi32(l, 2), one), _mm256_cmpeq_epi32(_mm256_and_si256(l, three), zero));
+        acc_l = _mm256_add_epi64(acc_l, _mm256_add_epi64(_mm256_and_si256(l, low32), _mm256_srli_epi64(l, 32)));
+        acc_pb = _mm256_add_epi64(acc_pb, _mm256_add_epi64(_mm256_and_si256(pbl, low32), _mm256_srli_epi64(pbl, 32)));
+        __m256i q0[4], q1[4], q2[4];
+        quads_avx2(a, b, p, la, q0);
+        quads_avx2(zero, l, _mm256_xor_si256(b, one), _mm256_xor_si256(a, one), q1);
+        quads_avx2(_mm256_sub_epi32(lb, l), lb, zero, l, q2);
+        __m256i y[12];
+        y[0] = _mm256_permute2x128_si256(q0[0], q1[0], 0x20), y[1] = _mm256_permute2x128_si256(q2[0], q0[1], 0x20);
+        y[2] = _mm256_permute2x128_si256(q1[1], q2[1], 0x20), y[3] = _mm256_permute2x128_si256(q0[2], q1[2], 0x20);
+        y[4] = _mm256_permute2x128_si256(q2[2], q0[3], 0x20), y[5] = _mm256_permute2x128_si256(q1[3], q2[3], 0x20);
+        y[6] = _mm256_permute2x128_si256(q0[0], q1[0], 0x31), y[7] = _mm256_permute2x128_si256(q2[0], q0[1], 0x31);
+        y[8] = _mm256_permute2x128_si256(q1[1], q2[1], 0x31), y[9] = _mm256_permute2x128_si256(q0[2], q1[2], 0x31);
+        y[10] = _mm256_permute2x128_si256(q2[2], q0[3], 0x31), y[11] = _mm256_permute2x128_si256(q1[3], q2[3], 0x31);
+        if (!run) {
+            sh = (uint32_t)((32u - (uint32_t)(reinterpret_cast<uintptr_t>(o) & 31u)) & 31u) / 8u;
+            if (sh) {
+                words_out_avx2(y[0], sh, o);
+                const int d = (int)(2u * sh);
+                rot = _mm256_and_si256(_mm256_add_epi32(_mm256_setr_epi32(0, 1, 2, 3, 4, 5, 6, 7), _mm256_set1_epi32(d)), _mm256_set1_epi32(7));
+                mask = _mm256_cmpgt_epi32(_mm256_setr_epi32(0, 1, 2, 3, 4, 5, 6, 7), _mm256_set1_epi32(7 - d));
+            }
+        }
+        if (sh == 0) {
+            __m256i* dst = reinterpret_cast<__m256i*>(o);
+            for (int k = 0; k < 12; ++k) _mm256_stream_si256(dst + k, y[k]);
+        } else {
+            __m256i* dst = reinterpret_cast<__m256i*>(o + sh);
+            __m256i prev = _mm256_permutevar8x32_epi32(y[0], rot);
+            if (run) _mm256_stream_si256(dst - 1, _mm256_blendv_epi8(carry, prev, mask));
+            for (int k = 0; k < 11; ++k) {
+                const __m256i next = _mm256_permutevar8x32_epi32(y[k + 1], rot);
+                _mm256_stream_si256(dst + k, _mm256_blendv_epi8(prev, next, mask));
+                prev = next;
+            }
+            carry = prev;
+        }
+        run = true;
+        o += 48;
+    }
+    if (run) words_out_avx2(carry, sh ? 4u - sh : 0u, o - (sh ? 4u - sh : 0u));
+    if (!write_span_scalar(j, len, n_reads, i, hi, o, t)) return false;
+    alignas(32) uint64_t wl[4], wp[4];
+    _mm256_store_si256(reinterpret_cast<__m256i*>(wl), acc_l);
+    _mm256_store_si256(reinterpret_cast<__m256i*>(wp), acc_pb);
+    const uint64_t sum_l = wl[0] + wl[1] + wl[2] + wl[3], sum_pb = wp[0] + wp[1] + wp[2] + wp[3];
+    s.l += t.l + 2 * sum_l;
+    s.b += t.b + 4 * sum_pb;
+    s.e += t.e + 2 * sum_pb;
+    return true;
+}
+
+#endif
+
+inline int vector_level() {
+#if defined(PHASM_HOME_AVX2)
+    return __builtin_cpu_supports("avx2") ? 2 : 0;
+#else
+    return 0;
+#endif
+}
+
+inline uint64_t count_chunk(const Recs& j, uint64_t lo, uint64_t hi, int level) {
+#if defined(PHASM_HOME_AVX2)
+    if (level >= 2 && j.sh_b) return count_chunk_avx2(j, lo, hi);
+#endif
+    (void)level;
+    return count_chunk_scalar(j, lo, hi);
+}
+
+inline bool write_chunk(const Recs& j, const uint32_t* len, uint32_t n_reads, uint64_t lo, uint64_t hi, void* out, Sums& s, int level) {
+#if defined(PHASM_HOME_AVX2)
+    if (level >= 2 && j.sh_b) return write_chunk_avx2(j, len, n_reads, lo, hi, out, s);
+#endif
+    (void)level;
+    return write_chunk_scalar(j, len, n_reads, lo, hi, out, s);
+}
+
+}
diff --git a/phasm_amd/csrc/kernels.hip.h b/phasm_amd/csrc/kernels.hip.h
--- a/phasm_amd/csrc/kernels.hip.h
+++ b/phasm_amd/csrc/kernels.hip.h
@@ -1984,12 +1984,9 @@
     if (k < cap) out[k] = Cand{cand_a[i], cand_p[i], b, 0u};
 }
 
-__global__ __launch_bounds__(256) void k_verify_flat(const uint64_t* __restrict__ words, const uint64_t* __restrict__ woff,
-                                                     const uint32_t* __restrict__ len, Cand* __restrict__ cands, uint32_t n,
-                                                     const uint32_t* __restrict__ exc_off, const uint32_t* __restrict__ exc_pos,
-                                                     const uint8_t* __restrict__ exc_byte) {
-    const uint32_t i = (blockIdx.x * blockDim.x + threadIdx.x) >> 6;
-    if (i >= n) return;
+__device__ inline void verify_flat_one(const uint64_t* __restrict__ words, const uint64_t* __restrict__ woff, const uint32_t* __restrict__ len,
+                                       Cand* __restrict__ cands, uint32_t i, const uint32_t* __restrict__ exc_off,
+                                       const uint32_t* __restrict__ exc_pos, const uint8_t* __restrict__ exc_byte) {
     const uint32_t lane = lane_id();
     const Cand c = cands[i];
     const uint32_t la = len[c.a], lb = len[c.b];
@@ -2007,6 +2004,75 @@
     bool any_bad = __any(bad);
     if (lane == 0 && !any_bad && exc_off && !exceptions_equal(exc_off, exc_pos, exc_byte, c.a, c.p, c.b, lb)) any_bad = true;
     if (lane == 0) cands[i].type = any_bad ? 0u : 2u;
+}
+
+__global__ __launch_bounds__(256) void k_verify_flat(const uint64_t* __restrict__ words, const uint64_t* __restrict__ woff,
+                                                     const uint32_t* __restrict__ len, Cand* __restrict__ cands, uint32_t n,
+                                                     const uint32_t* __restrict__ exc_off, const uint32_t* __restrict__ exc_pos,
+                                                     const uint8_t* __restrict__ exc_byte) {
+    const uint32_t i = (blockIdx.x * blockDim.x + threadIdx.x) >> 6;
+    if (i >= n) return;
+    verify_flat_one(words, woff, len, cands, i, exc_off, exc_pos, exc_byte);
+}
+
+__global__ __launch_bounds__(256) void k_verify_flat_dev(const uint64_t* __restrict__ words, const uint64_t* __restrict__ woff,
+                                                         const uint32_t* __restrict__ len, Cand* __restrict__ cands,
+                                                         const uint32_t* __restrict__ n_dev, uint32_t cap, uint32_t limit,
+                                                         const uint32_t* __restrict__ exc_off, const uint32_t* __restrict__ exc_pos,
+                                                         const uint8_t* __restrict__ exc_byte) {
+    const uint32_t n = *n_dev;
+    if (n > cap || n > limit) return;
+    const uint32_t waves = gridDim.x * (blockDim.x >> 6);
+    for (uint32_t i = (blockIdx.x * blockDim.x + threadIdx.x) >> 6; i < n; i += waves)
+        verify_flat_one(words, woff, len, cands, i, exc_off, exc_pos, exc_byte);
+}
+
+constexpr uint32_t DEFER_RECORDS_BLOCK = 1024;
+__global__ __launch_bounds__(DEFER_RECORDS_BLOCK) void k_defer_records(const Cand* __restrict__ cands, const uint32_t* __restrict__ n_dev,
+                                                                       uint32_t cap, uint32_t limit, Cand* __restrict__ out, uint32_t sh_b,
+                                                                       uint32_t sh_p, uint64_t* __restrict__ host_out) {
+    __shared__ uint32_t s_wave[DEFER_RECORDS_BLOCK / WAVE];
+    __shared__ uint32_t s_base;
+    const uint32_t n = *n_dev;
+    if (n > cap || n > limit) {
+        if (threadIdx.x == 0) {
+            host_out[0] = n;
+            host_out[1] = ~0ull;
+            host_out[2] = 0;
+        }
+        return;
+    }
+    if (threadIdx.x == 0) s_base = 0;
+    __syncthreads();
+    const uint32_t lane = lane_id(), wave = threadIdx.x >> 6;
+    uint64_t* out8 = reinterpret_cast<uint64_t*>(out);
+    for (uint32_t start = 0; start < n; start += DEFER_RECORDS_BLOCK) {
+        const uint32_t i = start + threadIdx.x;
+        Cand c = Cand{0u, 0u, 0u, 0u};
+        if (i < n) c = cands[i];
+        const bool v = c.type != 0u;
+        const uint64_t m = __ballot(v);
+        if (lane == 0) s_wave[wave] = (uint32_t)__popcll(m);
+        __syncthreads();
+        uint32_t at = s_base + (uint32_t)__popcll(m & ((1ull << lane) - 1ull));
+        for (uint32_t w = 0; w < wave; ++w) at += s_wave[w];
+        if (v) {
+            if (sh_b) out8[at] = pack_record(c.a, c.p, c.b, c.type, sh_b, sh_p);
+            else out[at] = c;
+        }
+        __syncthreads();
+        if (threadIdx.x == 0) {
+            uint32_t t = 0;
+            for (uint32_t w = 0; w < DEFER_RECORDS_BLOCK / WAVE; ++w) t += s_wave[w];
+            s_base += t;
+        }
+        __syncthreads();
+    }
+    if (threadIdx.x == 0) {
+        host_out[0] = n;
+        host_out[1] = s_base;
+        host_out[2] = 2ull * s_base;
+    }
 }
 
 __global__ void k_deferred_rowcnt(const Cand* __restrict__ cands, uint32_t n, uint32_t paired, uint8_t* __restrict__ rowcnt) {
```
